# HKUNLP/efficient-attention

Measured on AMD Instinct MI355X. Metric: attn fwd+bwd tokens/s per GPU at N=784, d=64; 1/2/4/8-GPU DDP scaling, higher is better.
Workload: dtype bf16; 1 GPU; lara attention layer fwd+bwd+SGD, x=[128,28,28,192] per GPU (N=784, h=3, d=64), bf16 autocast; attn=lara, global_batch=128, seq_len=784, heads=3, head_dim=64, parallelism=dp1, hipgraph=True, gemm_tunableop=False

## Files before the change

### efficient-attention_amd/csrc/ea_capi.hip

```cpp
#include <stdlib.h>
#include <cmath>
#include "ea_window.h"

namespace ea {
int window_fwd_dispatch(const WinP& p, int dtype, int D, hipStream_t st);
int window_bwd_dispatch(const WinP& p, const ea_geom& geom, const T4& outp, const float* biasT, int dtype, int D,
                        hipStream_t st);
}
#include "ea_landmark_params.h"
#include "ea_lara.h"
#include "ea_softmax.h"
#include "ea_lara_lmk.h"
#include "ea_lara_merge.h"
#include "ea_layernorm.h"
#include "ea_lara_segment.h"
#include "ea_scatter.h"
#include "ea_rows_mlp.h"
#include "ea_performer_f32.h"
#include "ea_kernelized.h"
#include "ea_f32_attn.h"
namespace ea {
int rows_mlp_dispatch(const RowsP& p, int D, int sides, int layer_norm, bool bwd, hipStream_t st);
int rows_mlp_blocks(int R, int D);
int lara_x_dispatch(int mode, const LaraP& p, int dtype, hipStream_t st);
int lara_y_dispatch(int mode, const LaraP& p, int dtype, hipStream_t st);
int lara_f_dispatch(int which, const LaraP& p, int dtype, hipStream_t st);
int pool2d_dispatch(bool bwd, int dtype, const void* x, long sb, long sh, long sn, float* mean, int B, int H, int gh, int gw,
                    int side, int D, hipStream_t st);
int linear_supported(int K, int NO);
int proj_rs_supported(int K, int NO);
int proj_rs_pool_supported(int K, int NO, int B, int gh, int gw, int r);
int proj_rs_dispatch(int dtype, const void* a, int a_f32, const float* w, const float* bias, void* y, void* a_cast, int rows,
                     long lda, long ldy, hipStream_t st, int B, int gh, int gw, int r, float* pq, float* pk, void* w_cast,
                     const void* wsw);
int w192_prepare_dispatch(int dtype, const float* wq, const float* wp, void* w16q, void* wsw, void* w16p, void* w16pT, hipStream_t st);
int dgrad_rs_supported(int K, int NO);
int dgrad_fin_launch(int dtype, const void* dqkv, long ldy, const void* qkv, long ldq, const void* w, int w_f32, void* dx, int dx_f32,
                     long ldx, int B, int gh, int gw, int pool_r, int C, float scale, const float* qbar, const float* uq,
                     const float* lse_t, const float* dpq, const float* dpk, hipStream_t st);
int dgrad_rs_dispatch(int dtype, const void* dy, const void* w, int w_f32, void* dx, int dx_f32, int rows, long ldy, long ldx,
                      hipStream_t st);
int linear_dispatch(int dtype, const void* a, int a_f32, const void* w, int w_mode, const float* bias, void* y, int y_f32,
                    void* a_cast, int rows, int K, int NO, long lda, long ldy, hipStream_t st);
int wgrad_slices(int rows, int M, int K);
int wgrad_pair_slices(int rows, int M1, int K1, int M2, int K2);
int wgrad_pair_dispatch(int dtype, int rows, const void* dy1, const void* x1, float* part1, float* db1, long ld1, int M1, int K1,
                        const void* dy2, const void* x2, float* part2, float* db2, long ld2, int M2, int K2, hipStream_t st);
int wgrad_dispatch(int dtype, const void* dy, const void* x, float* part, float* db_part, long part_ld, int rows, int M,
                   int K, hipStream_t st);
int part_sum_dispatch(const float* part, float* out, int S, int n, long ld, hipStream_t st);
int multi_sum_dispatch(int K, const float* const* part, const int* S, const int* n, const long long* ld, float* const* out,
                       hipStream_t st);
}

using namespace ea;

static bool t4_ok(const ea_t4* t, int D) {
  return t && t->ptr && ((uintptr_t)t->ptr % 16 == 0) && t->sb % 8 == 0 && t->sh % 8 == 0 &&
         t->sn % 8 == 0 && t->sn >= D;
}
static bool t4_ok32(const ea_t4* t, int D, int N) {
  return t4_ok(t, D) && (int64_t)N * t->sn < ((int64_t)1 << 31);
}
static bool geom_ok(const ea_geom* g) {
  return g && g->B > 0 && g->H > 0 && g->N > 0 && (g->D == 32 || g->D == 64 || g->D == 128) &&
         (g->dtype == EA_BF16 || g->dtype == EA_F16) && g->ext >= 0 && g->causal >= 0 && g->causal <= 2 && g->lm_base >= 0;
}
static Geo mk_geo(const ea_geom* g) {
  Geo G;
  G.N = g->N; G.attn2d = g->attn_2d; G.gh = g->attn_2d ? g->gh : 1; G.gw = g->attn_2d ? g->gw : g->N;
  return G;
}

extern "C" {

const char* ea_version(void) { return "ea_hip 0.1.0 gfx950"; }
int32_t ea_abi_version(void) { return 24; }

int32_t ea_window_bias_ld(const ea_geom* g) {
  WinTiling t;
  if (!geom_ok(g) || win_tiling(*g, t, false) != EA_OK) return EA_E_BADARG;
  return t.biasLd;
}
int32_t ea_window_keep_ld(const ea_geom* g) {
  WinTiling t;
  if (!geom_ok(g) || win_tiling(*g, t, false) != EA_OK) return EA_E_BADARG;
  return t.biasLd + t.nCT * 16;
}
int32_t ea_window_bwd_parts(const ea_geom* g) {
  WinTiling t;
  if (!geom_ok(g) || win_tiling(*g, t, true) != EA_OK) return EA_E_BADARG;
  return t.parts_total;
}
int32_t ea_window_bwd_needs_bias_t(const ea_geom* g) {
  WinTiling t;
  if (!geom_ok(g) || win_tiling(*g, t, true) != EA_OK) return EA_E_BADARG;
  int any = 0;
  win_bwd_launches(*g, t, [&](const WinTiling& tl) { any |= window_bwd_lds(tl, g->D, true, true) > WIN_LDS_MAX; });
  return any;
}
int32_t ea_window_bwd_bias_parts(const ea_geom* g) {
  WinTiling t;
  if (!geom_ok(g) || win_tiling(*g, t, true) != EA_OK) return EA_E_BADARG;
  return win_bwd_bias_parts(*g, t);
}
int32_t ea_window_bwd_acc_slices(const ea_geom* g) {
  WinTiling t;
  if (!geom_ok(g) || win_tiling(*g, t, true) != EA_OK) return EA_E_BADARG;
  return win_bwd_acc_slices(t);
}
int32_t ea_window_bwd_query_blocks(const ea_geom* g) {
  WinTiling t;
  if (!geom_ok(g) || win_tiling(*g, t, true) != EA_OK) return EA_E_BADARG;
  return t.qsplit;
}

static int fill_win(const ea_geom* g, WinP& p, bool backward) {
  if (!geom_ok(g)) return EA_E_BADARG;
  int rc = win_tiling(*g, p.t, backward);
  if (rc != EA_OK) return rc;
  if (g->L < 0 || g->L > 64) return EA_E_UNSUPPORTED;
  p.G = mk_geo(g);
  p.B = g->B; p.H = g->H; p.L = g->L; p.w = g->window; p.e = g->ext;
  p.causal = g->causal; p.chunk = g->chunk; p.lm_base = g->causal == 2 ? g->lm_base : 0;
  p.scale = g->scale;
  p.scale_log2 = g->scale * LOG2E;
  return EA_OK;
}

int ea_window_attn_fwd(const ea_geom* g, const ea_t4* q, const ea_t4* k, const ea_t4* v,
                       const float* lk, const float* lv, const float* bias, const uint8_t* mask,
                       const ea_t4* out, float* lse, const uint8_t* keep, float keep_scale, void* stream) {
  WinP p = {};
  int rc = fill_win(g, p, false);
  if (rc != EA_OK) return rc;
  if (keep && !g->causal) return EA_E_UNSUPPORTED;
  p.keep = keep; p.keep_scale = keep_scale; p.keep_ld = p.t.biasLd + p.t.nCT * 16;
  if (!t4_ok(q, g->D) || !t4_ok(k, g->D) || !t4_ok(v, g->D) || !t4_ok(out, g->D) || !lse) return EA_E_BADARG;
  if (g->L > 0 && (!lk || !lv)) return EA_E_BADARG;
  p.q = mk(q); p.k = mk(k); p.v = mk(v); p.o = mk(out);
  p.lk = lk; p.lv = lv; p.bias = bias; p.mask = mask; p.lse = lse;
  return window_fwd_dispatch(p, g->dtype, g->D, (hipStream_t)stream);
}

int ea_window_attn_bwd(const ea_geom* g, const ea_t4* q, const ea_t4* k, const ea_t4* v,
                       const float* lk, const float* lv, const float* bias, const uint8_t* mask,
                       const ea_t4* out, const ea_t4* dout, const float* lse,
                       const ea_t4* dq, const ea_t4* dk, const ea_t4* dv,
                       float* dlk_part, float* dlv_part, float* dbias_part,
                       float* dk_acc, float* dv_acc, const float* bias_t,
                       const uint8_t* keep, float keep_scale, const float* dlse, void* stream) {
  WinP p = {};
  int rc = fill_win(g, p, true);
  if (rc != EA_OK) return rc;
  p.dlse = dlse;
  if (keep && !g->causal) return EA_E_UNSUPPORTED;
  p.keep = keep; p.keep_scale = keep_scale; p.keep_ld = p.t.biasLd + p.t.nCT * 16;
  const int N = g->N;
  if (!t4_ok32(q, g->D, N) || !t4_ok32(k, g->D, N) || !t4_ok32(v, g->D, N) || !t4_ok32(dout, g->D, N) ||
      !t4_ok32(out, g->D, N) || (win_bwd_acc_slices(p.t) > 0 && (!dk_acc || !dv_acc)) || !t4_ok32(dq, g->D, N) ||
// ... 1205 lines not shown
extern "C" {

int32_t ea_linear_supported(int32_t in_features, int32_t out_features) { return linear_supported(in_features, out_features); }

int ea_linear(int32_t dtype, int32_t rows, int32_t in_features, int32_t out_features, const void* a, int32_t a_f32,
              int64_t lda, const void* w, const float* bias, void* y, int32_t y_f32, int64_t ldy, void* a_cast,
              void* stream) {
  if (!a || !w || !y || ((uintptr_t)a & 15) || ((uintptr_t)w & 15) || ((uintptr_t)y & 15) || ((uintptr_t)bias & 15) ||
      ((uintptr_t)a_cast & 15))
    return EA_E_BADARG;
  if (lda < in_features || ldy < out_features || (lda & 7) || (ldy & 7)) return EA_E_BADARG;
  return linear_dispatch(dtype, a, a_f32, w, 0, bias, y, y_f32, a_cast, rows, in_features, out_features, (long)lda,
                         (long)ldy, (hipStream_t)stream);
}

int ea_linear_w32(int32_t dtype, int32_t rows, int32_t in_features, int32_t out_features, const void* a, int32_t a_f32,
                  int64_t lda, const float* w, int32_t w_transposed, const float* bias, void* y, int32_t y_f32, int64_t ldy,
                  void* a_cast, void* stream) {
  if (!a || !w || !y || ((uintptr_t)a & 15) || ((uintptr_t)w & 15) || ((uintptr_t)y & 15) || ((uintptr_t)bias & 15) ||
      ((uintptr_t)a_cast & 15))
    return EA_E_BADARG;
  if (lda < in_features || ldy < out_features || (lda & 7) || (ldy & 7)) return EA_E_BADARG;
  static const bool rs_on = !(getenv("EA_PROJ_RS") && getenv("EA_PROJ_RS")[0] == '0');
  if (rs_on && !w_transposed && !y_f32 && rows >= 65536 && proj_rs_supported(in_features, out_features))
    return proj_rs_dispatch(dtype, a, a_f32, w, bias, y, a_cast, rows, (long)lda, (long)ldy, (hipStream_t)stream, 0, 0, 0, 0,
                            nullptr, nullptr, nullptr, nullptr);
  return linear_dispatch(dtype, a, a_f32, w, w_transposed ? 2 : 1, bias, y, y_f32, a_cast, rows, in_features, out_features,
                         (long)lda, (long)ldy, (hipStream_t)stream);
}

int32_t ea_linear_dgrad_supported(int32_t in_features, int32_t out_features) {
  return dgrad_rs_supported(out_features, in_features);
}

int ea_linear_dgrad(int32_t dtype, int32_t rows, int32_t in_features, int32_t out_features, const void* dy, int64_t ldy,
                    const void* w, int32_t w_f32, void* dx, int32_t dx_f32, int64_t ldx, void* stream) {
  if (!dy || !w || !dx || ((uintptr_t)dy & 15) || ((uintptr_t)w & 15) || ((uintptr_t)dx & 15)) return EA_E_BADARG;
  if (rows < 0 || ldy < out_features || ldx < in_features || (ldy & 7) || (ldx & 3) || (!dx_f32 && (ldx & 7))) return EA_E_BADARG;
  if (!dgrad_rs_supported(out_features, in_features)) return EA_E_UNSUPPORTED;
  if ((int64_t)rows * ldy >= ((int64_t)1 << 40)) return EA_E_BADARG;
  return dgrad_rs_dispatch(dtype, dy, w, w_f32, dx, dx_f32, rows, (long)ldy, (long)ldx, (hipStream_t)stream);
}

int ea_linear_dgrad_finish(int32_t dtype, int32_t B, int32_t gh, int32_t gw, int32_t pool_r, int32_t C, float scale,
                           void* dqkv, int64_t ldy, const void* qkv, int64_t ldq, const void* w, int32_t w_f32, void* dx,
                           int32_t dx_f32, int64_t ldx, const float* qbar, const float* uq, const float* lse_t,
                           const float* dpq, const float* dpk, void* stream) {
  if (!dqkv || !w || !dx || ((uintptr_t)dqkv & 15) || ((uintptr_t)w & 15) || ((uintptr_t)dx & 15) || ((uintptr_t)qkv & 15))
    return EA_E_BADARG;
  if (B <= 0 || gh <= 0 || gw <= 0 || ldy < 576 || ldx < 192 || (ldy & 7) || (ldx & 3) || (!dx_f32 && (ldx & 7))) return EA_E_BADARG;
  if ((dpq == nullptr) != (dpk == nullptr)) return EA_E_BADARG;
  if (dpq && (pool_r <= 0 || gh % pool_r || gw % pool_r)) return EA_E_BADARG;
  if (uq && (!qkv || !qbar || !lse_t || ldq < 192 || (ldq & 7) || C <= 0)) return EA_E_BADARG;
  if (uq && C > 64) return EA_E_UNSUPPORTED;
  if (!uq && !dpq) return EA_E_BADARG;
  if ((int64_t)B * gh * gw >= ((int64_t)1 << 31)) return EA_E_BADARG;
  return dgrad_fin_launch(dtype, dqkv, (long)ldy, qkv, (long)ldq, w, w_f32, dx, dx_f32, (long)ldx, B, gh, gw, pool_r, C, scale,
                          qbar, uq, lse_t, dpq, dpk, (hipStream_t)stream);
}

int32_t ea_linear_pool_supported(int32_t in_features, int32_t out_features, int32_t B, int32_t gh, int32_t gw, int32_t r) {
  return proj_rs_pool_supported(in_features, out_features, B, gh, gw, r);
}

int ea_linear_w32_pool(int32_t dtype, int32_t B, int32_t gh, int32_t gw, int32_t r, int32_t in_features, int32_t out_features,
                       const void* a, int32_t a_f32, int64_t lda, const float* w, const float* bias, void* y, int64_t ldy,
                       void* a_cast, float* pooled_q, float* pooled_k, void* w_cast, void* stream) {
  if (!a || !w || !y || !pooled_q || !pooled_k || ((uintptr_t)a & 15) || ((uintptr_t)w & 15) || ((uintptr_t)y & 15) ||
      ((uintptr_t)bias & 15) || ((uintptr_t)a_cast & 15) || ((uintptr_t)pooled_q & 15) || ((uintptr_t)pooled_k & 15) ||
      ((uintptr_t)w_cast & 15))
    return EA_E_BADARG;
  if (lda < in_features || ldy < out_features || (lda & 7) || (ldy & 7)) return EA_E_BADARG;
  if (!proj_rs_pool_supported(in_features, out_features, B, gh, gw, r)) return EA_E_UNSUPPORTED;
  return proj_rs_dispatch(dtype, a, a_f32, w, bias, y, a_cast, B * gh * gw, (long)lda, (long)ldy, (hipStream_t)stream, B, gh, gw,
                          r, pooled_q, pooled_k, w_cast, nullptr);
}

int ea_linear_w192_prepare(int32_t dtype, const float* wq, const float* wp, void* w16q, void* wq_sw, void* w16p, void* w16pT,
                           void* stream) {
  if (!wq || !w16q || !wq_sw || ((uintptr_t)wq & 15) || ((uintptr_t)wp & 15) || ((uintptr_t)w16q & 15) || ((uintptr_t)wq_sw & 15) ||
      ((uintptr_t)w16p & 15) || ((uintptr_t)w16pT & 15))
    return EA_E_BADARG;
  if (wp && (!w16p || !w16pT)) return EA_E_BADARG;
  return w192_prepare_dispatch(dtype, wq, wp, w16q, wq_sw, w16p, w16pT, (hipStream_t)stream);
}

int ea_linear_wsw(int32_t dtype, int32_t rows, int32_t B, int32_t gh, int32_t gw, int32_t r, const void* a, int32_t a_f32, int64_t lda,
                  const void* wq_sw, const float* bias, void* y, int64_t ldy, void* a_cast, float* pooled_q, float* pooled_k,
                  void* stream) {
  if (!a || !wq_sw || !y || ((uintptr_t)a & 15) || ((uintptr_t)wq_sw & 15) || ((uintptr_t)y & 15) || ((uintptr_t)bias & 15) ||
      ((uintptr_t)a_cast & 15) || ((uintptr_t)pooled_q & 15) || ((uintptr_t)pooled_k & 15))
    return EA_E_BADARG;
  if (lda < 192 || ldy < 576 || (lda & 7) || (ldy & 7) || rows <= 0) return EA_E_BADARG;
  if (r != 0) {
    if (!pooled_q || !pooled_k || rows != B * gh * gw) return EA_E_BADARG;
    if (!proj_rs_pool_supported(192, 576, B, gh, gw, r)) return EA_E_UNSUPPORTED;
  }
  return proj_rs_dispatch(dtype, a, a_f32, nullptr, bias, y, a_cast, rows, (long)lda, (long)ldy, (hipStream_t)stream, B, gh, gw, r,
                          r ? pooled_q : nullptr, r ? pooled_k : nullptr, nullptr, wq_sw);
}

}

static T4s mks(const ea_t4* t) {
  T4s r;
  r.p = t ? (char*)t->ptr : nullptr;
  r.sb = t ? t->sb : 0; r.sh = t ? t->sh : 0; r.sn = t ? t->sn : 0;
  return r;
}
static int fill_sb(const ea_sb_geom* g, SbP& p) {
  if (!g || g->B <= 0 || g->H <= 0 || g->N <= 0 || g->window <= 0 || (g->dtype != EA_BF16 && g->dtype != EA_F16))
    return EA_E_BADARG;
  if (g->D != 64 || g->M <= 0 || g->M > 64) return EA_E_UNSUPPORTED;
  p.B = g->B; p.H = g->H; p.N = g->N; p.M = g->M; p.w = g->window;
  p.G.N = g->N; p.G.attn2d = g->attn_2d; p.G.gh = g->attn_2d ? g->gh : 1; p.G.gw = g->attn_2d ? g->gw : g->N;
  if (g->attn_2d) {
    if (g->gh % g->window || g->gw % g->window || g->gh * g->gw != g->N) return EA_E_BADARG;
    p.Wq = g->window * g->window;
    p.nwin = (g->gh / g->window) * (g->gw / g->window);
  } else {
    if (g->N % g->window) return EA_E_BADARG;
    p.Wq = g->window;
    p.nwin = g->N / g->window;
  }
  if (p.Wq > 64) return EA_E_UNSUPPORTED;
  p.a = 1.f / sqrtf(sqrtf(64.f));
  p.b = 0.5f / sqrtf(64.f);
  p.lconst = 0.5f * logf((float)g->M);
  p.wpb = 1;
  for (int d = 2; d <= 4; ++d)
    if (p.nwin % d == 0) p.wpb = d;
  return EA_OK;
}
static int fill_sb_stats(const ea_sb_geom* g, LaraP& p) {
  ea_perf_geom pg;
  pg.B = g->B; pg.H = g->H; pg.N = g->N; pg.D = g->D; pg.dtype = g->dtype; pg.M = g->M;
  int rc = fill_perf(&pg, p, true);
  if (rc != EA_OK) return rc;
  p.ratio = 1.f; p.feps = 0.f; p.stab_per_feature = 1;
  return EA_OK;
}

extern "C" {

int32_t ea_scatter_parts(const ea_sb_geom* g) {
  LaraP p = {};
  if (!g || fill_sb_stats(g, p) != EA_OK) return EA_E_BADARG;
  return p.nsplit * lara_nsub(p.NCT);
}

int ea_scatter_kmax(const ea_sb_geom* g, const ea_t4* k, const uint8_t* mask, const float* W, float* p_ml, void* stream) {
  LaraP p = {};
  if (!g) return EA_E_BADARG;
  int rc = fill_sb_stats(g, p);
  if (rc != EA_OK) return rc;
  if (!t4_ok(k, g->D) || !W || !p_ml) return EA_E_BADARG;
  p.k = mkl(k); p.mask = mask; p.omega = W; p.p_ml = p_ml;
  return lara_y_dispatch(LY_PMAX, p, g->dtype, (hipStream_t)stream);
}

int ea_scatter_kv(const ea_sb_geom* g, const ea_t4* k, const ea_t4* v, const uint8_t* mask, const float* W,
                  const float* mx, float* p_ml, float* p_kv, void* stream) {
  LaraP p = {};
  if (!g) return EA_E_BADARG;
  int rc = fill_sb_stats(g, p);
  if (rc != EA_OK) return rc;
  if (!t4_ok(k, g->D) || !t4_ok(v, g->D) || !W || !mx || !p_ml || !p_kv) return EA_E_BADARG;
// ... 778 lines not shown
```

### efficient-attention_amd/csrc/ea_common.h

```cpp
#pragma once
#include <hip/hip_runtime.h>
#include <stdint.h>
#include "../../include/ea_hip.h"

#ifdef EA_PROFILE
#include <stdio.h>
#include <algorithm>
#include <vector>
#define EA_STAMP(p, i) do { if (threadIdx.x == 0 && blockIdx.x == 0 && (p).prof) (p).prof[i] = (long long)__builtin_readcyclecounter(); } while (0)
#define EA_BLK(p, e) do { if (threadIdx.x == 0 && (p).prof && blockIdx.x < 8192) (p).prof[128 + 2 * blockIdx.x + (e)] = (long long)wall_clock64(); } while (0)
#define EA_BLKX(p, e) do { if (threadIdx.x == 0 && (p).prof && blockIdx.x < 8192) (p).prof[128 + 2 * 8192 + 2 * blockIdx.x + (e)] = (long long)wall_clock64(); } while (0)
namespace ea {
struct ProfReport {
  static constexpr int NW = 128 + 4 * 8192;
  long long* d = nullptr; hipStream_t st; const char* name; int mode;
  long long* arm(hipStream_t s, const char* nm, int md) {
    static long long* buf = nullptr;
    if (!buf) hipMalloc(&buf, NW * sizeof(long long));
    hipMemsetAsync(buf, 0, NW * sizeof(long long), s);
    d = buf; st = s; name = nm; mode = md;
    return buf;
  }
  ~ProfReport() {
    if (!d) return;
    std::vector<long long> h(NW);
    hipStreamSynchronize(st);
    hipMemcpy(h.data(), d, NW * sizeof(long long), hipMemcpyDeviceToHost);
    fprintf(stderr, "%s mode %d:", name, mode);
    long long prev = h[0];
    for (int i = 1; i < 128; ++i) if (h[i]) { fprintf(stderr, " [%d]%lld", i, h[i] - prev); prev = h[i]; }
    fprintf(stderr, " total %lld\n", prev - h[0]);
    std::vector<long long> b, e, dur;
    for (int i = 0; i < 8192; ++i) if (h[128 + 2 * i] && h[129 + 2 * i]) { b.push_back(h[128 + 2 * i]); e.push_back(h[129 + 2 * i]); dur.push_back(h[129 + 2 * i] - h[128 + 2 * i]); }
    if (!b.empty()) {
      const long long t0 = *std::min_element(b.begin(), b.end());
      std::vector<long long> bs(b), es(e), ds(dur);
      for (auto& x : bs) x -= t0; for (auto& x : es) x -= t0;
      std::sort(bs.begin(), bs.end()); std::sort(es.begin(), es.end()); std::sort(ds.begin(), ds.end());
      const size_t n = bs.size();
      fprintf(stderr, "  %zu blocks (10 ns ticks): start p50 %lld p90 %lld max %lld | dur min %lld p50 %lld p90 %lld max %lld | end p50 %lld max %lld\n",
              n, bs[n / 2], bs[n * 9 / 10], bs[n - 1], ds[0], ds[n / 2], ds[n * 9 / 10], ds[n - 1], es[n / 2], es[n - 1]);
      {
        std::vector<long long> pro, epi;
        for (int i = 0; i < 8192; ++i) {
          const long long b0 = h[128 + 2 * i], e0 = h[129 + 2 * i], x0 = h[128 + 2 * 8192 + 2 * i], x1 = h[129 + 2 * 8192 + 2 * i];
          if (b0 && e0 && x0 && x1) { pro.push_back(x0 - b0); epi.push_back(e0 - x1); }
        }
        if (!pro.empty()) {
          std::sort(pro.begin(), pro.end()); std::sort(epi.begin(), epi.end());
          const size_t m = pro.size();
          fprintf(stderr, "  prologue p10 %lld p50 %lld p90 %lld | epilogue p10 %lld p50 %lld p90 %lld\n", pro[m / 10], pro[m / 2], pro[m * 9 / 10], epi[m / 10], epi[m / 2], epi[m * 9 / 10]);
        }
      }
      fprintf(stderr, "  start deciles:");
      for (int q = 1; q <= 10; ++q) fprintf(stderr, " %lld", bs[(n * q) / 10 - 1]);
      fprintf(stderr, " | dur deciles:");
      for (int q = 1; q <= 10; ++q) fprintf(stderr, " %lld", ds[(n * q) / 10 - 1]);
      fprintf(stderr, " | end deciles:");
      for (int q = 1; q <= 10; ++q) fprintf(stderr, " %lld", es[(n * q) / 10 - 1]);
      fprintf(stderr, "\n");
    }
  }
};
}
#else
#define EA_STAMP(p, i) do { } while (0)
#define EA_BLK(p, e) do { } while (0)
#define EA_BLKX(p, e) do { } while (0)
#endif


namespace ea {

constexpr int EA_MAX_DEV = 64;
inline int ea_cur_device() {
  int dev = 0;
  if (hipGetDevice(&dev) != hipSuccess || dev < 0 || dev >= EA_MAX_DEV) dev = 0;
  return dev;
}
inline int ea_device_cus() {
  static int n[EA_MAX_DEV] = {};
  const int dev = ea_cur_device();
  if (!n[dev]) {
    hipDeviceProp_t prop;
    int v = 0;
    if (hipGetDeviceProperties(&prop, dev) == hipSuccess) v = prop.multiProcessorCount;
// ... 105 lines not shown
template <int G> EA_DEV float group_sum(float v) {
  static_assert(G == 4 || G == 8 || G == 16, "group_sum: 4, 8 or 16 lanes");
  v += dpp_mov<0xB1>(v);
  v += dpp_mov<0x4E>(v);
  if (G >= 8) v += dpp_mov<0x141>(v);
  if (G >= 16) v += dpp_mov<0x128>(v);
  return v;
}
template <int S> EA_DEV float stride_sum(float v) {
  static_assert(S == 4 || S == 8 || S == 16, "stride_sum: stride 4, 8 or 16");
  if (S <= 8) v += dpp_mov<0x128>(v);
  if (S <= 4) v += dpp_mov<0x124>(v);
  return quad_sum(v);
}
template <int S> EA_DEV float stride_max(float v) {
  static_assert(S == 4 || S == 8 || S == 16, "stride_max: stride 4, 8 or 16");
  if (S <= 8) v = fmaxf(v, dpp_mov<0x128>(v));
  if (S <= 4) v = fmaxf(v, dpp_mov<0x124>(v));
  return quad_max(v);
}
EA_DEV float fast_rcp(float x) { return __builtin_amdgcn_rcpf(x); }
EA_DEV float wave_sum(float v) {
#pragma unroll
  for (int o = 32; o > 0; o >>= 1) v += __shfl_xor(v, o);
  return v;
}

static __device__ __attribute__((aligned(64))) char ea_trash[512 * 64];
EA_DEV char* ea_trash_line() { return ea_trash + threadIdx.x * 64; }

#ifdef EA_NT_LOADS
EA_DEV u32x4 ldg16(const void* p) { return __builtin_nontemporal_load(reinterpret_cast<const u32x4*>(p)); }
#else
EA_DEV u32x4 ldg16(const void* p) { return *reinterpret_cast<const u32x4*>(p); }
#endif
#ifdef EA_NT_STORES
EA_DEV void stg16(void* p, u32x4 v) { __builtin_nontemporal_store(v, reinterpret_cast<u32x4*>(p)); }
#else
EA_DEV void stg16(void* p, u32x4 v) { *reinterpret_cast<u32x4*>(p) = v; }
#endif
EA_DEV u32x4 lds16(const char* p) { return *reinterpret_cast<const u32x4*>(p); }
EA_DEV void sts16(char* p, u32x4 v) { *reinterpret_cast<u32x4*>(p) = v; }

struct Geo {
  int N, attn2d, gh, gw;
};
EA_DEV int part_token(const Geo& G, int part, int slot, int side, int ext) {
  if (G.attn2d) {
    const int t = side + 2 * ext;
    const int per_row = G.gw / side;
    const int p1 = part / per_row, p2 = part - p1 * per_row;
    const int i = slot / t, j = slot - i * t;
    const int y = p1 * side - ext + i, x = p2 * side - ext + j;
    return (y >= 0 && y < G.gh && x >= 0 && x < G.gw) ? y * G.gw + x : -1;
  }
  const int tok = part * side - ext + slot;
  return (tok >= 0 && tok < G.N) ? tok : -1;
}

template <int D> EA_DEV int lds_off(int row, int chunk16) {
  constexpr int CPR = D / 8;
  constexpr int SW = CPR >= 8 ? 7 : CPR - 1;
  return row * (D * 2) + ((chunk16 ^ (row & SW)) << 4);
}

template <int D> struct LaneOff {
  static constexpr int ROWB = D * 2, CPR = D / 8, KS = D / 32, DT = D / 16, DQ = D / 4;
  static constexpr int SW = CPR >= 8 ? 7 : CPR - 1;
  int plain[KS];
  int tr[DT];
  EA_DEV void init(int lane) {
    const int g = lane >> 4, li = lane & 15;
#pragma unroll
    for (int ks = 0; ks < KS; ++ks) plain[ks] = li * ROWB + (((g * KS + ks) ^ (li & SW)) << 4);
    const int r = 4 * g + (li >> 2);
#pragma unroll
    for (int dt = 0; dt < DT; ++dt) {
      const int colb = (DQ * (li & 3) + 4 * dt) * 2;
      tr[dt] = r * ROWB + ((((colb >> 4)) ^ (r & SW)) << 4) + (colb & 15);
    }
  }
};

EA_DEV int phi2(int row) { return (((row >> 1) & 3) << 1) | ((row ^ (row >> 3)) & 1); }
template <int D> EA_DEV int lds_off2(int row, int chunk16) {
  static_assert(D == 64, "lds_off2: 128-byte rows only");
  return row * (D * 2) + ((chunk16 ^ phi2(row)) << 4);
}
template <int D> struct LaneOff2 {
  static constexpr int ROWB = D * 2, KS = D / 32, DT = D / 16;
  int plain[KS];
  int tr[DT];
  EA_DEV void init(int lane) {
    const int g = lane >> 4, li = lane & 15;
#pragma unroll
    for (int ks = 0; ks < KS; ++ks) plain[ks] = lds_off2<D>(li, g * KS + ks);
    const int r = 4 * g + (li >> 2);
#pragma unroll
    for (int dt = 0; dt < DT; ++dt) tr[dt] = lds_off2<D>(r, 2 * dt + ((li & 3) >> 1)) + 8 * (li & 1);
  }
};
template <int W> EA_DEV void quad_transpose(uint32_t (&x)[4][W]);
template <> EA_DEV void quad_transpose<2>(uint32_t (&x)[4][2]) {
  asm volatile("s_nop 15\n\tv_permlane32_swap_b32 %0, %4\n\tv_permlane32_swap_b32 %2, %6\n\t"
               "v_permlane32_swap_b32 %1, %5\n\tv_permlane32_swap_b32 %3, %7"
               : "+v"(x[0][0]), "+v"(x[0][1]), "+v"(x[1][0]), "+v"(x[1][1]), "+v"(x[2][0]), "+v"(x[2][1]), "+v"(x[3][0]), "+v"(x[3][1]));
  asm volatile("s_nop 1\n\tv_permlane16_swap_b32 %0, %2\n\tv_permlane16_swap_b32 %4, %6\n\t"
               "v_permlane16_swap_b32 %1, %3\n\tv_permlane16_swap_b32 %5, %7"
               : "+v"(x[0][0]), "+v"(x[0][1]), "+v"(x[1][0]), "+v"(x[1][1]), "+v"(x[2][0]), "+v"(x[2][1]), "+v"(x[3][0]), "+v"(x[3][1]));
}
template <> EA_DEV void quad_transpose<4>(uint32_t (&x)[4][4]) {
  asm volatile("s_nop 15\n\t"
               "v_permlane32_swap_b32 %0, %8\n\tv_permlane32_swap_b32 %4, %12\n\t"
               "v_permlane32_swap_b32 %1, %9\n\tv_permlane32_swap_b32 %5, %13\n\t"
               "v_permlane32_swap_b32 %2, %10\n\tv_permlane32_swap_b32 %6, %14\n\t"
               "v_permlane32_swap_b32 %3, %11\n\tv_permlane32_swap_b32 %7, %15"
               : "+v"(x[0][0]), "+v"(x[0][1]), "+v"(x[0][2]), "+v"(x[0][3]), "+v"(x[1][0]), "+v"(x[1][1]), "+v"(x[1][2]), "+v"(x[1][3]),
                 "+v"(x[2][0]), "+v"(x[2][1]), "+v"(x[2][2]), "+v"(x[2][3]), "+v"(x[3][0]), "+v"(x[3][1]), "+v"(x[3][2]), "+v"(x[3][3]));
  asm volatile("s_nop 1\n\t"
               "v_permlane16_swap_b32 %0, %4\n\tv_permlane16_swap_b32 %8, %12\n\t"
               "v_permlane16_swap_b32 %1, %5\n\tv_permlane16_swap_b32 %9, %13\n\t"
               "v_permlane16_swap_b32 %2, %6\n\tv_permlane16_swap_b32 %10, %14\n\t"
               "v_permlane16_swap_b32 %3, %7\n\tv_permlane16_swap_b32 %11, %15"
               : "+v"(x[0][0]), "+v"(x[0][1]), "+v"(x[0][2]), "+v"(x[0][3]), "+v"(x[1][0]), "+v"(x[1][1]), "+v"(x[1][2]), "+v"(x[1][3]),
                 "+v"(x[2][0]), "+v"(x[2][1]), "+v"(x[2][2]), "+v"(x[2][3]), "+v"(x[3][0]), "+v"(x[3][1]), "+v"(x[3][2]), "+v"(x[3][3]));
}
EA_DEV void quad_transpose_f32(const f32x4* acc, float* f) {
  uint32_t x[4][4];
#pragma unroll
  for (int s = 0; s < 4; ++s)
#pragma unroll
    for (int r = 0; r < 4; ++r) {
      const float t = acc[s][r];
      x[s][r] = __builtin_bit_cast(uint32_t, t);
    }
  quad_transpose<4>(x);
#pragma unroll
  for (int s = 0; s < 4; ++s)
#pragma unroll
    for (int r = 0; r < 4; ++r) f[4 * s + r] = __builtin_bit_cast(float, x[s][r]);
}
template <typename E> EA_DEV void quad_transpose_pack(const f32x4* acc, float mul, u32x4& o0, u32x4& o1) {
  uint32_t x[4][2];
#pragma unroll
  for (int s = 0; s < 4; ++s) {
    x[s][0] = pack2<E>(acc[s][0] * mul, acc[s][1] * mul);
    x[s][1] = pack2<E>(acc[s][2] * mul, acc[s][3] * mul);
  }
  quad_transpose<2>(x);
  o0 = u32x4{x[0][0], x[0][1], x[1][0], x[1][1]};
  o1 = u32x4{x[2][0], x[2][1], x[3][0], x[3][1]};
}

template <int D> struct TileL {
  static constexpr bool NEWTR = (D == 64);
  static EA_DEV int off(int row, int chunk16) {
    if constexpr (NEWTR) return lds_off2<D>(row, chunk16);
    else return lds_off<D>(row, chunk16);
  }
};
template <int D> EA_DEV int tile_tr(int r, int li, int dt) {
  const int colb = TileL<D>::NEWTR ? (16 * dt + 4 * (li & 3)) * 2 : ((D / 4) * (li & 3) + 4 * dt) * 2;
  return TileL<D>::off(r, colb >> 4) + (colb & 15);
}
template <int D> struct LaneOffSel { typedef LaneOff<D> type; };
template <> struct LaneOffSel<64> { typedef LaneOff2<64> type; };
template <int D> EA_DEV int acc_chan(int dt, int g) { return TileL<D>::NEWTR ? 16 * dt + 4 * g : (D / 4) * g + 4 * dt; }

}
```

### efficient-attention_amd/csrc/ea_dgrad_rs.hip

```cpp
#include <stdlib.h>
#include "ea_common.h"

namespace ea {

struct DgP {
  const char* dy;
  const char* w;
  char* dx;
  int rows, ntiles;
  long ldy, ldx;
  long long* prof;
};

constexpr int DG_K = 576, DG_NO = 192, DG_WAVES = 12, DG_TOK = 32, DG_KT = DG_K / 32, DG_SLABS = DG_K / 64;
constexpr int DG_TILE = DG_SLABS * DG_TOK * 128;
constexpr int DG_PIECE = 32 * DG_NO * 2;
constexpr int DG_LDS = 2 * DG_TILE;

EA_DEV int dg_off(int slab, int tok, int chunk16) { return slab * (DG_TOK * 128) + lds_off2<64>(tok, chunk16); }

template <typename E, bool WF32, bool OF32>
__global__ __launch_bounds__(DG_WAVES * 64, 3) void dgrad_rs_kernel(const DgP p) {
  extern __shared__ __attribute__((aligned(16))) char smem[];
  char* const tile0 = smem;
  char* const tile1 = smem + DG_TILE;
  const int tid = threadIdx.x, lane = tid & 63, g = lane >> 4, li = lane & 15;
  const int wave = __builtin_amdgcn_readfirstlane(tid >> 6);
  int s_tok[3], s_ch[3];
#pragma unroll
  for (int i = 0; i < 3; ++i) {
    const int s = tid + i * (DG_WAVES * 64);
    s_tok[i] = s / 72;
    s_ch[i] = s - s_tok[i] * 72;
  }
  u32x4 nb[3];
  auto issue = [&](int t) {
#pragma unroll
    for (int i = 0; i < 3; ++i) {
      const int tok = min(t * DG_TOK + s_tok[i], p.rows - 1);
      nb[i] = ldg16(p.dy + ((size_t)tok * p.ldy + s_ch[i] * 8) * 2);
    }
  };
  int t = blockIdx.x;
  if (t < p.ntiles) issue(t);
  typename E::x8 wr[DG_KT];
  {
    const int o_l = tid / 24, c = tid - o_l * 24;
    const int rho = ((o_l >> 2) & 1) * 16 + (o_l >> 3) * 4 + (o_l & 3);
    const int wofs = rho * (DG_NO * 2) + c * 16;
    const int rofs = (4 * g + (li >> 2)) * (DG_NO * 2) + (16 * wave + 4 * (li & 3)) * 2;
    constexpr int BATCH = 6;
#pragma unroll
    for (int pb = 0; pb < DG_KT; pb += BATCH) {
      u32x4 raw[BATCH][WF32 ? 2 : 1];
#pragma unroll
      for (int j = 0; j < BATCH; ++j) {
        const size_t e = (size_t)(32 * (pb + j) + o_l) * DG_NO + c * 8;
        if constexpr (WF32) {
          raw[j][0] = ldg16(p.w + e * 4);
          raw[j][1] = ldg16(p.w + e * 4 + 16);
        } else {
          raw[j][0] = ldg16(p.w + e * 2);
        }
      }
#pragma unroll
      for (int j = 0; j < BATCH; ++j) {
        u32x4 w8;
        if constexpr (WF32) {
          const f32x4 lo = __builtin_bit_cast(f32x4, raw[j][0]), hi = __builtin_bit_cast(f32x4, raw[j][1]);
          const float f[8] = {lo[0], lo[1], lo[2], lo[3], hi[0], hi[1], hi[2], hi[3]};
          w8 = pack8<E>(f);
        } else {
          w8 = raw[j][0];
        }
        char* img = tile1 + ((pb + j) & 1) * DG_PIECE;
        sts16(img + wofs, w8);
        __syncthreads();
        wr[pb + j] = as_x8<E>(E::tr4(img + rofs), E::tr4(img + rofs + 16 * (DG_NO * 2)));
      }
    }
  }
  int buf = 0;
  for (; t < p.ntiles; t += gridDim.x, buf ^= 1) {
    char* const tb = buf ? tile1 : tile0;
#pragma unroll
    for (int i = 0; i < 3; ++i) sts16(tb + dg_off(s_ch[i] >> 3, s_tok[i], s_ch[i] & 7), nb[i]);
    issue(min(t + (int)gridDim.x, p.ntiles - 1));
    __syncthreads();
    f32x4 acc[2][2];
#pragma unroll
    for (int rt = 0; rt < 2; ++rt) acc[rt][0] = acc[rt][1] = f32x4{0.f, 0.f, 0.f, 0.f};
#pragma unroll
    for (int ks = 0; ks < DG_KT; ++ks) {
      const int slab = ks >> 1;
      const typename E::x8 b0 = as_x8<E>(lds16(tb + dg_off(slab, li, 4 * (ks & 1) + g)));
      const typename E::x8 b1 = as_x8<E>(lds16(tb + dg_off(slab, 16 + li, 4 * (ks & 1) + g)));
      acc[0][ks & 1] = E::mma(wr[ks], b0, acc[0][ks & 1]);
      acc[1][ks & 1] = E::mma(wr[ks], b1, acc[1][ks & 1]);
    }
#pragma unroll
    for (int rt = 0; rt < 2; ++rt) {
      const int tok = min(t * DG_TOK + 16 * rt + li, p.rows - 1);
      const f32x4 v = acc[rt][0] + acc[rt][1];
      const int col = 16 * wave + 4 * g;
      if constexpr (OF32) {
        *reinterpret_cast<f32x4*>(p.dx + ((size_t)tok * p.ldx + col) * 4) = v;
      } else {
        *reinterpret_cast<u32x2*>(p.dx + ((size_t)tok * p.ldx + col) * 2) = u32x2{pack2<E>(v[0], v[1]), pack2<E>(v[2], v[3])};
      }
    }
  }
}

struct DgFinP {
  DgP d;
  const char* qkv;
  long ldq;
  const float *qbar, *uq, *lse_t;
  const float *dpq, *dpk;
  int ntok, gw, pool_r, cw, L, C;
  float pool_inv, scale, scale_log2;
  int splits, tps, nunits;
  unsigned m_gw, m_r;
  int cps;
  unsigned m_cw;
};

constexpr int DG_QT = 3 * DG_TOK * 128;
constexpr int DG_LMR = 64 * 128;
constexpr int DG_FIN_LDS = 2 * DG_TILE + 2 * DG_QT + 6 * DG_LMR + 3 * 64 * 4;

template <typename E, bool WF32, bool OF32, bool HAS_T, bool POOL, int PR>
__global__ __launch_bounds__(DG_WAVES * 64, 3) void dgrad_fin_kernel(const DgFinP p) {
  static_assert(PR == 0 || (POOL && (PR == 2 || PR == 4)), "cell-major order needs 2 x 2 or 4 x 4 pooling cells");
  constexpr int TPC = PR * PR, CPT = PR ? DG_TOK / (PR * PR) : 1;
  extern __shared__ __attribute__((aligned(16))) char smem[];
  char* const tile0 = smem;
  char* const tile1 = smem + DG_TILE;
  char* const qt0 = smem + 2 * DG_TILE;
  char* const R1 = qt0 + 2 * DG_QT;
  char* const R2 = R1 + 3 * DG_LMR;
  float* const LS = reinterpret_cast<float*>(R2 + 3 * DG_LMR);
  const int tid = threadIdx.x, lane = tid & 63, g = lane >> 4, li = lane & 15;
  const int wave = __builtin_amdgcn_readfirstlane(tid >> 6);
  constexpr bool pool = POOL;
  EA_BLK(p.d, 0);
  typename E::x8 wr[DG_KT];
  {
    const int o_l = tid / 24, c = tid - o_l * 24;
    const int rho = ((o_l >> 2) & 1) * 16 + (o_l >> 3) * 4 + (o_l & 3);
    const int wofs = rho * (DG_NO * 2) + c * 16;
    const int rofs = (4 * g + (li >> 2)) * (DG_NO * 2) + (16 * wave + 4 * (li & 3)) * 2;
    constexpr int BATCH = 6;
#pragma unroll
    for (int pb = 0; pb < DG_KT; pb += BATCH) {
      u32x4 raw[BATCH][WF32 ? 2 : 1];
#pragma unroll
      for (int j = 0; j < BATCH; ++j) {
        const size_t e = (size_t)(32 * (pb + j) + o_l) * DG_NO + c * 8;
        if constexpr (WF32) {
          raw[j][0] = ldg16(p.d.w + e * 4);
          raw[j][1] = ldg16(p.d.w + e * 4 + 16);
        } else {
          raw[j][0] = ldg16(p.d.w + e * 2);
        }
      }
#pragma unroll
      for (int j = 0; j < BATCH; ++j) {
        u32x4 w8;
        if constexpr (WF32) {
          const f32x4 lo = __builtin_bit_cast(f32x4, raw[j][0]), hi = __builtin_bit_cast(f32x4, raw[j][1]);
          const float f[8] = {lo[0], lo[1], lo[2], lo[3], hi[0], hi[1], hi[2], hi[3]};
          w8 = pack8<E>(f);
        } else {
          w8 = raw[j][0];
        }
        char* img = tile1 + ((pb + j) & 1) * DG_PIECE;
        sts16(img + wofs, w8);
        __syncthreads();
        wr[pb + j] = as_x8<E>(E::tr4(img + rofs), E::tr4(img + rofs + 16 * (DG_NO * 2)));
      }
    }
  }
  typename LaneOffSel<64>::type lo;
  lo.init(lane);
  const int fh = wave >> 2, fnt = (wave >> 1) & 1, fdh = wave & 1;
  int buf = 0;
  EA_BLKX(p.d, 0);
  for (int u = blockIdx.x; u < p.nunits; u += gridDim.x) {
    const int b = u / p.splits, sp = u - b * p.splits;
    const int n0 = PR ? sp * p.cps : sp * p.tps, n1 = PR ? min(p.L, n0 + p.cps) : min(p.ntok, n0 + p.tps);
    const size_t row0 = (size_t)b * p.ntok;
    const int ntile = PR ? (n1 - n0 + CPT - 1) / CPT : (n1 - n0 + DG_TOK - 1) / DG_TOK;
    auto slot_cell = [&](int t, int r) { return min(n0 + t * CPT + r / (TPC ? TPC : 1), n1 - 1); };
    auto dup = [&](int t, int r) {
      if constexpr (PR == 0) return n0 + t * DG_TOK + r > n1 - 1;
      else return n0 + t * CPT + r / (TPC ? TPC : 1) > n1 - 1;
    };
    auto trash_line = [&]() {
      int t_ = tid;
      asm volatile("" : "+v"(t_));
      return ea_trash + (t_ & 511) * 64;
    };
    auto tok_of = [&](int t, int r) {
      if constexpr (PR == 0) {
        return min(n0 + t * DG_TOK + r, n1 - 1);
      } else {
        const int cell = slot_cell(t, r), w = r % TPC;
        const int cy = (int)__umulhi((unsigned)cell, p.m_cw), cx = cell - cy * p.cw;
        return (cy * PR + w / PR) * p.gw + cx * PR + w % PR;
      }
    };
    auto cell_of_tok = [&](int tok) {
      const int y = (int)__umulhi((unsigned)tok, p.m_gw), x = tok - y * p.gw;
      return (int)__umulhi((unsigned)y, p.m_r) * p.cw + (int)__umulhi((unsigned)x, p.m_r);
    };
    auto cell_of = [&](int t, int r) {
      if constexpr (PR == 0) return cell_of_tok(tok_of(t, r));
      else return slot_cell(t, r);
    };
    u32x4 nb[3], nq;
    f32x4 npk[2], npq[2];
    auto issue = [&](int t, int s_tok, int s_c) {
      const int tok = tok_of(t, s_tok);
      const char* rowp = p.d.dy + ((row0 + tok) * p.d.ldy + s_c * 8) * 2;
      nb[0] = ldg16(rowp);
      nb[1] = ldg16(rowp + 192 * 2);
      nb[2] = ldg16(rowp + 384 * 2);
      if constexpr (HAS_T) nq = ldg16(p.qkv + ((row0 + tok) * p.ldq + s_c * 8) * 2);
#ifdef EA_DGF_NOPOOLREAD
      npk[0] = npk[1] = npq[0] = npq[1] = f32x4{0.f, 0.f, 0.f, 0.f};
// ... 82 lines not shown
        const float* src = p.dpq + ((size_t)(b * 3 + fh) * p.L + cell_of(t, 16 * fnt + li)) * 64 + 4 * g;
#pragma unroll
        for (int j = 0; j < 2; ++j) pq4[j] = *reinterpret_cast<const f32x4*>(src + 16 * (2 * fdh + j));
      }
      issue(min(t + 1, ntile - 1), s_tok, s_c);
      __syncthreads();
      if constexpr (HAS_T) {
        const char* R1h = R1 + fh * DG_LMR;
        const char* R2h = R2 + fh * DG_LMR;
        const float* LSh = LS + fh * 64;
        typename E::x8 f1[2];
#pragma unroll
        for (int ks = 0; ks < 2; ++ks) f1[ks] = as_x8<E>(lds16(qb + dg_off(fh, 16 * fnt + li, g * 2 + ks)));
        f32x4 acc[2] = {f32x4{0.f, 0.f, 0.f, 0.f}, f32x4{0.f, 0.f, 0.f, 0.f}};
#pragma unroll
        for (int kk = 0; kk < 2; ++kk) {
          uint32_t pw[4];
#pragma unroll
          for (int c2 = 0; c2 < 2; ++c2) {
            const int ct = 2 * kk + c2;
            f32x4 tt = {0.f, 0.f, 0.f, 0.f};
#pragma unroll
            for (int ks = 0; ks < 2; ++ks) tt = E::mma(as_x8<E>(lds16(R2h + TileL<64>::off(ct * 16 + li, g * 2 + ks))), f1[ks], tt);
            const f32x4 ls = *reinterpret_cast<const f32x4*>(LSh + ct * 16 + 4 * g);
            pw[2 * c2] = pack2<E>(fast_exp2(tt[0] * p.scale_log2 - ls[0]), fast_exp2(tt[1] * p.scale_log2 - ls[1]));
            pw[2 * c2 + 1] = pack2<E>(fast_exp2(tt[2] * p.scale_log2 - ls[2]), fast_exp2(tt[3] * p.scale_log2 - ls[3]));
          }
          const u32x4 p1 = {pw[0], pw[1], pw[2], pw[3]};
#pragma unroll
          for (int j = 0; j < 2; ++j) {
            const char* r1 = R1h + (32 * kk) * 128 + (fdh ? lo.tr[2 + j] : lo.tr[j]);
            acc[j] = E::mma(as_x8<E>(E::tr4(r1), E::tr4(r1 + 16 * 128)), as_x8<E>(p1), acc[j]);
          }
        }
#pragma unroll
        for (int j = 0; j < 2; ++j) {
          const int dt = 2 * fdh + j;
          char* a = tb + dg_off(fh, 16 * fnt + li, 2 * dt + (g >> 1)) + (g & 1) * 8;
          const u32x2 old = *reinterpret_cast<const u32x2*>(a);
          float o4[4];
          unpack2<E>(old[0], o4[0], o4[1]);
          unpack2<E>(old[1], o4[2], o4[3]);
#pragma unroll
          for (int r = 0; r < 4; ++r) o4[r] = o4[r] - acc[j][r] * p.scale + pq4[j][r] * p.pool_inv;
          *reinterpret_cast<u32x2*>(a) = u32x2{pack2<E>(o4[0], o4[1]), pack2<E>(o4[2], o4[3])};
        }
        __syncthreads();
        stg16(dup(t, s_tok) ? trash_line() : const_cast<char*>(p.d.dy) + ((row0 + tok_of(t, s_tok)) * p.d.ldy + s_c * 8) * 2,
              lds16(tb + dg_off(s_c >> 3, s_tok, s_c & 7)));
      }
      f32x4 acc[2][2];
#pragma unroll
      for (int rt = 0; rt < 2; ++rt) acc[rt][0] = acc[rt][1] = f32x4{0.f, 0.f, 0.f, 0.f};
#pragma unroll
      for (int ks = 0; ks < DG_KT; ++ks) {
        const int slab = ks >> 1;
        const typename E::x8 b0 = as_x8<E>(lds16(tb + dg_off(slab, li, 4 * (ks & 1) + g)));
        const typename E::x8 b1 = as_x8<E>(lds16(tb + dg_off(slab, 16 + li, 4 * (ks & 1) + g)));
        acc[0][ks & 1] = E::mma(wr[ks], b0, acc[0][ks & 1]);
        acc[1][ks & 1] = E::mma(wr[ks], b1, acc[1][ks & 1]);
      }
      int li_x = lane;
      asm volatile("" : "+v"(li_x));
      li_x &= 15;
#pragma unroll
      for (int rt = 0; rt < 2; ++rt) {
        const size_t row = row0 + tok_of(t, 16 * rt + li_x);
        const bool dpx = dup(t, 16 * rt + li_x);
        const f32x4 v = acc[rt][0] + acc[rt][1];
        const int col = 16 * wave + 4 * g;
        if constexpr (OF32) {
          *reinterpret_cast<f32x4*>(dpx ? trash_line() : p.d.dx + (row * p.d.ldx + col) * 4) = v;
        } else {
          *reinterpret_cast<u32x2*>(dpx ? trash_line() : p.d.dx + (row * p.d.ldx + col) * 2) = u32x2{pack2<E>(v[0], v[1]), pack2<E>(v[2], v[3])};
        }
      }
    }
    if constexpr (HAS_T) __syncthreads();
  }
  EA_BLKX(p.d, 1);
  EA_BLK(p.d, 1);
}

int dgrad_rs_supported(int K, int NO) { return K == DG_K && NO == DG_NO; }

int dgrad_rs_dispatch(int dtype, const void* dy, const void* w, int w_f32, void* dx, int dx_f32, int rows, long ldy, long ldx,
                      hipStream_t st) {
  if (rows <= 0) return EA_OK;
  DgP p = {};
  p.dy = (const char*)dy; p.w = (const char*)w; p.dx = (char*)dx;
  p.rows = rows; p.ntiles = (rows + DG_TOK - 1) / DG_TOK; p.ldy = ldy; p.ldx = ldx;
  int grid = ea_device_cus();
  if (grid > p.ntiles) grid = p.ntiles;
  const dim3 g((unsigned)grid), b(DG_WAVES * 64);
#define EA_DG_LAUNCH(E_, WF_, OF_)                                                        \
  do {                                                                                    \
    EA_SET_LDS_ONCE((&dgrad_rs_kernel<E_, WF_, OF_>), DG_LDS);                            \
    hipLaunchKernelGGL((dgrad_rs_kernel<E_, WF_, OF_>), g, b, DG_LDS, st, p);             \
  } while (0)
#define EA_DG_SEL(E_)                                                                     \
  do {                                                                                    \
    if (w_f32) { if (dx_f32) EA_DG_LAUNCH(E_, true, true); else EA_DG_LAUNCH(E_, true, false); }   \
    else { if (dx_f32) EA_DG_LAUNCH(E_, false, true); else EA_DG_LAUNCH(E_, false, false); }       \
  } while (0)
  if (dtype == EA_BF16) EA_DG_SEL(BF16);
  else if (dtype == EA_F16) EA_DG_SEL(F16);
  else return EA_E_BADARG;
#undef EA_DG_SEL
#undef EA_DG_LAUNCH
  return (int)hipGetLastError();
}

int dgrad_fin_dispatch(int dtype, const DgFinP& p0, int w_f32, int dx_f32, bool has_t, int pr, hipStream_t st) {
  DgFinP p = p0;
  if (p.d.rows <= 0) return EA_OK;
  int grid = ea_device_cus();
  if (grid > p.nunits) grid = p.nunits;
  const dim3 g((unsigned)grid), b(DG_WAVES * 64);
#ifdef EA_PROFILE
  ProfReport rep;
  p.d.prof = rep.arm(st, "dgrad_fin", pr);
#endif
#define EA_DF_LAUNCH(E_, WF_, OF_, T_, P_, R_)                                                    \
  do {                                                                                            \
    EA_SET_LDS_ONCE((&dgrad_fin_kernel<E_, WF_, OF_, T_, P_, R_>), DG_FIN_LDS);                   \
    hipLaunchKernelGGL((dgrad_fin_kernel<E_, WF_, OF_, T_, P_, R_>), g, b, DG_FIN_LDS, st, p);    \
  } while (0)
#define EA_DF_SEL3(E_, WF_, OF_, T_)                                                          \
  do {                                                                                        \
    if (pr == 4) EA_DF_LAUNCH(E_, WF_, OF_, T_, true, 4);                                     \
    else if (pr == 2) EA_DF_LAUNCH(E_, WF_, OF_, T_, true, 2);                                \
    else EA_DF_LAUNCH(E_, WF_, OF_, T_, true, 0);                                             \
  } while (0)
#define EA_DF_SEL2(E_, WF_, OF_)                                                              \
  do {                                                                                        \
    if (has_t && p.dpq) EA_DF_SEL3(E_, WF_, OF_, true);                                       \
    else if (has_t) EA_DF_LAUNCH(E_, WF_, OF_, true, false, 0);                               \
    else EA_DF_SEL3(E_, WF_, OF_, false);                                                     \
  } while (0)
#define EA_DF_SEL(E_)                                                                     \
  do {                                                                                    \
    if (w_f32) { if (dx_f32) EA_DF_SEL2(E_, true, true); else EA_DF_SEL2(E_, true, false); }   \
    else { if (dx_f32) EA_DF_SEL2(E_, false, true); else EA_DF_SEL2(E_, false, false); }       \
  } while (0)
  if (dtype == EA_BF16) EA_DF_SEL(BF16);
  else if (dtype == EA_F16) EA_DF_SEL(F16);
  else return EA_E_BADARG;
#undef EA_DF_SEL
#undef EA_DF_SEL2
#undef EA_DF_SEL3
#undef EA_DF_LAUNCH
  return (int)hipGetLastError();
}

int dgrad_fin_launch(int dtype, const void* dqkv, long ldy, const void* qkv, long ldq, const void* w, int w_f32, void* dx, int dx_f32,
                     long ldx, int B, int gh, int gw, int pool_r, int C, float scale, const float* qbar, const float* uq,
                     const float* lse_t, const float* dpq, const float* dpk, hipStream_t st) {
  DgFinP p = {};
  p.d.dy = (const char*)dqkv; p.d.w = (const char*)w; p.d.dx = (char*)dx;
  p.ntok = gh * gw;
  p.d.rows = B * p.ntok; p.d.ntiles = 0; p.d.ldy = ldy; p.d.ldx = ldx;
  p.qkv = (const char*)qkv; p.ldq = ldq;
  p.qbar = qbar; p.uq = uq; p.lse_t = lse_t; p.dpq = dpq; p.dpk = dpk;
  p.gw = gw; p.pool_r = dpq ? pool_r : 1; p.cw = gw / p.pool_r; p.L = (gh / p.pool_r) * p.cw; p.C = C;
  p.pool_inv = 1.f / (float)(p.pool_r * p.pool_r); p.scale = scale; p.scale_log2 = scale * LOG2E;
  p.m_gw = (unsigned)((1ull << 32) / (unsigned)gw) + 1u; p.m_r = (unsigned)((1ull << 32) / (unsigned)p.pool_r) + 1u;
  const int cus = ea_device_cus();
  int splits = (cus + B - 1) / B;
  if (splits < 1) splits = 1;
  int tps = ((p.ntok + splits - 1) / splits + DG_TOK - 1) / DG_TOK * DG_TOK;
  if (tps < 2 * DG_TOK) tps = 2 * DG_TOK;
  p.tps = tps;
  p.splits = (p.ntok + tps - 1) / tps;
  static const bool cells_on = !(getenv("EA_DGF_CELLS") && getenv("EA_DGF_CELLS")[0] == '0');
  int pr = 0;
  if (dpq && cells_on && (pool_r == 2 || pool_r == 4) && gh % pool_r == 0 && gw % pool_r == 0) {
    pr = pool_r;
    const int cpt = DG_TOK / (pr * pr);
    int cps = ((p.L + splits - 1) / splits + cpt - 1) / cpt * cpt;
    if (cps < 2 * cpt) cps = 2 * cpt;
    p.cps = cps;
    p.splits = (p.L + cps - 1) / cps;
    p.m_cw = (unsigned)((1ull << 32) / (unsigned)p.cw) + 1u;
  }
  p.nunits = B * p.splits;
  return dgrad_fin_dispatch(dtype, p, w_f32, dx_f32, uq != nullptr, pr, st);
}

}
```

### efficient-attention_amd/csrc/ea_proj_rs.hip

```cpp
#include "ea_common.h"

namespace ea {

struct RsP {
  const char* a;
  const float* w;
  const float* bias;
  char* y;
  char* a_cast;
  char* w_cast;
  int rows, ntiles;
  long lda, ldy;
  float *pq, *pk;
  int gw, cw, Lc, ntok, ncell;
  unsigned m_Lc, m_cw;
  long long* prof;
  const char* wsw;
};

constexpr int RS_K = 192, RS_NO = 576, RS_WAVES = 12, RS_TOK = 32, RS_KT = RS_K / 32, RS_SLABS = RS_K / 64;

EA_DEV int rs_off(int slab, int tok, int chunk16) { return slab * (RS_TOK * 128) + lds_off2<64>(tok, chunk16); }

EA_DEV int rs_col(int wave, int j, int li) {
  const int c0 = 48 * wave;
  return j == 2 ? c0 + 32 + li : c0 + 8 * (li >> 2) + (li & 3) + 4 * j;
}

template <typename E, bool AF32, int POOL, bool WSW>
__global__ __launch_bounds__(RS_WAVES * 64, 3) void proj_rs_kernel(const RsP p) {
  __shared__ __attribute__((aligned(16))) char tile[2][RS_SLABS * RS_TOK * 128];
  __shared__ __attribute__((aligned(16))) float bias_s[RS_NO];
  const int tid = threadIdx.x, lane = tid & 63, g = lane >> 4, li = lane & 15;
  const int wave = __builtin_amdgcn_readfirstlane(tid >> 6);
  const int st_tok = tid / 24, st_c = tid - st_tok * 24;
  constexpr int PR = POOL == 16 ? 4 : 2;
  auto cell_of = [&](int t, int s, int& img, int& cl) {
    const int cell = min(t * (RS_TOK / (POOL ? POOL : 1)) + s / (POOL ? POOL : 1), p.ncell - 1);
    img = (int)__umulhi((unsigned)cell, p.m_Lc);
    cl = cell - img * p.Lc;
  };
  auto tok_of = [&](int t, int s) {
    if constexpr (POOL == 0) {
      return min(t * RS_TOK + s, p.rows - 1);
    } else {
      int img, cl;
      cell_of(t, s, img, cl);
      const int cy = (int)__umulhi((unsigned)cl, p.m_cw), cx = cl - cy * p.cw;
      const int w = s % POOL, dy = w / PR, dx = w % PR;
      return img * p.ntok + (cy * PR + dy) * p.gw + cx * PR + dx;
    }
  };
  u32x4 nb[AF32 ? 2 : 1];
  auto issue = [&](int t) {
    const int tok = tok_of(t, st_tok);
    const char* ap = p.a + (size_t)tok * p.lda * (AF32 ? 4 : 2) + st_c * (AF32 ? 32 : 16);
    nb[0] = ldg16(ap);
    if constexpr (AF32) nb[1] = ldg16(ap + 16);
  };
  int t = blockIdx.x;
  EA_BLK(p, 0);
  if (t < p.ntiles) issue(t);
  typename E::x8 wr[3][RS_KT];
  for (int i = tid; i < RS_NO; i += RS_WAVES * 64) bias_s[i] = p.bias ? E::to_f(E::from_f(p.bias[i])) : 0.f;
  if constexpr (WSW) {
#pragma unroll
    for (int j = 0; j < 3; ++j)
#pragma unroll
      for (int ks = 0; ks < RS_KT; ++ks)
        wr[j][ks] = as_x8<E>(ldg16(p.wsw + ((size_t)((wave * 3 + j) * RS_KT + ks) * 64 + lane) * 16));
  } else {
    const int col[3] = {rs_col(wave, 0, li), rs_col(wave, 1, li), rs_col(wave, 2, li)};
#pragma unroll
    for (int j = 0; j < 3; ++j)
#pragma unroll
      for (int ks = 0; ks < RS_KT; ++ks) {
        const float* s = p.w + (size_t)col[j] * RS_K + ks * 32 + 8 * g;
        const f32x4 lo = *reinterpret_cast<const f32x4*>(s), hi = *reinterpret_cast<const f32x4*>(s + 4);
        const float f[8] = {lo[0], lo[1], lo[2], lo[3], hi[0], hi[1], hi[2], hi[3]};
        wr[j][ks] = as_x8<E>(pack8<E>(f));
        if (p.w_cast && (unsigned)((wave * 3 + j) * RS_KT + ks) % gridDim.x == blockIdx.x)
          stg16(p.w_cast + ((size_t)col[j] * RS_K + ks * 32 + 8 * g) * 2, __builtin_bit_cast(u32x4, wr[j][ks]));
      }
  }
  const int slab_s = st_c >> 3, ch_s = st_c & 7;
  constexpr int NC = POOL ? RS_TOK / POOL : 1;
  constexpr int XB = 8 * RS_K * 2;
  __shared__ __attribute__((aligned(16))) char xbar[POOL ? 2 : 1][POOL ? 2 * XB : 16];
  const int pc0 = 48 * wave;
  auto pool_x = [&](int b_) {
    const int slab = wave >> 2, dt = wave & 3;
    const char* tb = tile[b_] + slab * (RS_TOK * 128);
    const int r_ = 4 * g + (li >> 2);
    const int off = lds_off2<64>(r_, 2 * dt + ((li & 3) >> 1)) + 8 * (li & 1);
    const typename E::x8 a = as_x8<E>(E::tr4(tb + off), E::tr4(tb + 16 * 128 + off));
    const uint32_t one = (uint32_t)E::from_f(1.f) * 0x00010001u;
    const uint32_t lo_on = (POOL == 16 ? li == 0 : li == g) ? one : 0u, hi_on = (POOL == 16 ? li == 1 : li == 4 + g) ? one : 0u;
    const typename E::x8 pat = as_x8<E>(u32x4{lo_on, lo_on, hi_on, hi_on});
    const f32x4 d = E::mma(a, pat, f32x4{0.f, 0.f, 0.f, 0.f});
    float hi[4], lo[4];
#pragma unroll
    for (int r = 0; r < 4; ++r) {
      const float v = d[r] * (1.f / (POOL ? POOL : 1));
      hi[r] = E::to_f(E::from_f(v));
      lo[r] = v - hi[r];
    }
    if (li < NC) {
      char* dst = xbar[b_] + li * (RS_K * 2) + (64 * slab + 16 * dt + 4 * g) * 2;
      *reinterpret_cast<u32x2*>(dst) = u32x2{pack2<E>(hi[0], hi[1]), pack2<E>(hi[2], hi[3])};
      *reinterpret_cast<u32x2*>(dst + XB) = u32x2{pack2<E>(lo[0], lo[1]), pack2<E>(lo[2], lo[3])};
    }
  };
  auto pool_out = [&](int tp, int b_) {
    if (wave >= 8) return;
    f32x4 pa[3] = {f32x4{0.f, 0.f, 0.f, 0.f}, f32x4{0.f, 0.f, 0.f, 0.f}, f32x4{0.f, 0.f, 0.f, 0.f}};
    const char* xb = xbar[b_] + min(li, NC - 1) * (RS_K * 2);
#pragma unroll
    for (int ks = 0; ks < RS_KT; ++ks) {
      const typename E::x8 bh = as_x8<E>(lds16(xb + (4 * ks + g) * 16));
      const typename E::x8 bl = as_x8<E>(lds16(xb + XB + (4 * ks + g) * 16));
#pragma unroll
      for (int j = 0; j < 3; ++j) {
        pa[j] = E::mma(wr[j][ks], bh, pa[j]);
        pa[j] = E::mma(wr[j][ks], bl, pa[j]);
      }
    }
    const int cell = tp * NC + li;
    if (li < NC && cell < p.ncell) {
      const int img = (int)__umulhi((unsigned)cell, p.m_Lc), cl = cell - img * p.Lc;
      const int cols[3] = {pc0 + 8 * g, pc0 + 8 * g + 4, pc0 + 32 + 4 * g};
#pragma unroll
      for (int j = 0; j < 3; ++j) {
        const int side = wave >> 2, hc = cols[j] - side * RS_K, head = hc >> 6, ch = hc & 63;
        float* dst = (side ? p.pk : p.pq) + ((size_t)(img * 3 + head) * p.Lc + cl) * 64 + ch;
        *reinterpret_cast<f32x4*>(dst) = pa[j] + *reinterpret_cast<const f32x4*>(bias_s + cols[j]);
      }
    }
  };
  int buf = 0, tprev = -1;
  EA_BLKX(p, 0);
  for (; t < p.ntiles; tprev = t, t += gridDim.x, buf ^= 1) {
    {
      u32x4 w8;
      if constexpr (AF32) {
        const f32x4 lo = __builtin_bit_cast(f32x4, nb[0]), hi = __builtin_bit_cast(f32x4, nb[1]);
        const float f[8] = {lo[0], lo[1], lo[2], lo[3], hi[0], hi[1], hi[2], hi[3]};
        w8 = pack8<E>(f);
      } else {
        w8 = nb[0];
      }
      sts16(tile[buf] + rs_off(slab_s, st_tok, ch_s), w8);
      if (AF32 && p.a_cast) {
        const int tok = tok_of(t, st_tok);
        stg16(p.a_cast + ((size_t)tok * RS_K + st_c * 8) * 2, w8);
      }
    }
    if (t + (int)gridDim.x < p.ntiles) issue(t + gridDim.x);
    __syncthreads();
#ifndef EA_RS_NOPOOLMATH
    if constexpr (POOL > 0) pool_x(buf);
#endif
    f32x4 acc[3][2];
#pragma unroll
    for (int j = 0; j < 3; ++j) acc[j][0] = acc[j][1] = f32x4{0.f, 0.f, 0.f, 0.f};
#pragma unroll
    for (int ks = 0; ks < RS_KT; ++ks) {
      const int slab = ks >> 1;
      const typename E::x8 b0 = as_x8<E>(lds16(tile[buf] + rs_off(slab, li, 4 * (ks & 1) + g)));
      const typename E::x8 b1 = as_x8<E>(lds16(tile[buf] + rs_off(slab, 16 + li, 4 * (ks & 1) + g)));
#pragma unroll
      for (int j = 0; j < 3; ++j) {
        acc[j][0] = E::mma(wr[j][ks], b0, acc[j][0]);
        acc[j][1] = E::mma(wr[j][ks], b1, acc[j][1]);
      }
    }
    const int c0 = 48 * wave;
    const f32x4 bv0 = *reinterpret_cast<const f32x4*>(bias_s + c0 + 8 * g), bv1 = *reinterpret_cast<const f32x4*>(bias_s + c0 + 8 * g + 4);
    const f32x4 bv2 = *reinterpret_cast<const f32x4*>(bias_s + c0 + 32 + 4 * g);
    u32x2 third[2];
#pragma unroll
    for (int rt = 0; rt < 2; ++rt) {
      const int tok = tok_of(t, 16 * rt + li);
      char* yp = p.y + ((size_t)tok * p.ldy + c0) * 2;
      const f32x4 v0 = acc[0][rt] + bv0, v1 = acc[1][rt] + bv1, v2 = acc[2][rt] + bv2;
      u32x4 o;
      o[0] = pack2<E>(v0[0], v0[1]); o[1] = pack2<E>(v0[2], v0[3]);
      o[2] = pack2<E>(v1[0], v1[1]); o[3] = pack2<E>(v1[2], v1[3]);
      stg16(yp + 16 * g, o);
      third[rt] = u32x2{pack2<E>(v2[0], v2[1]), pack2<E>(v2[2], v2[3])};
    }
    asm volatile("s_nop 1\n\tv_permlane16_swap_b32 %0, %2\n\tv_permlane16_swap_b32 %1, %3"
                 : "+v"(third[0][0]), "+v"(third[0][1]), "+v"(third[1][0]), "+v"(third[1][1]));
    {
      const int tok = tok_of(t, 16 * (g & 1) + li);
      const u32x4 o = {third[0][0], third[0][1], third[1][0], third[1][1]};
      stg16(p.y + ((size_t)tok * p.ldy + c0 + 32 + 8 * (g >> 1)) * 2, o);
    }
#ifndef EA_RS_NOPOOLMATH
    if constexpr (POOL > 0) {
      if (tprev >= 0) pool_out(tprev, buf ^ 1);
    }
#endif
  }
  EA_BLKX(p, 1);
  if constexpr (POOL > 0) {
    if (tprev >= 0) {
      __syncthreads();
      pool_out(tprev, buf ^ 1);
    }
  }
  EA_BLK(p, 1);
}

int proj_rs_supported(int K, int NO) { return K == RS_K && NO == RS_NO; }

static unsigned rs_magic(int d) { return (unsigned)((1ull << 32) / (unsigned)d) + 1u; }

int proj_rs_pool_supported(int K, int NO, int B, int gh, int gw, int r) {
  if (K != RS_K || NO != RS_NO || (r != 2 && r != 4) || B <= 0 || gh <= 0 || gw <= 0 || gh % r || gw % r) return 0;
  const long Lc = (long)(gh / r) * (gw / r), ncell = (long)B * Lc;
  return ncell * Lc < (1l << 32) && (long)B * gh * gw < (1l << 31);
}

template <typename E>
__global__ __launch_bounds__(256) void w192_prepare_kernel(const float* __restrict__ wq, const float* __restrict__ wp,
                                                            char* __restrict__ w16q, char* __restrict__ wsw,
                                                            char* __restrict__ w16p, char* __restrict__ w16pT) {
  constexpr int NQ = RS_WAVES * 3 * RS_KT * 64, NP = RS_K * RS_K / 8;
  const int i = blockIdx.x * 256 + threadIdx.x;
  if (i < NQ) {
    const int lane = i & 63, pc = i >> 6, ks = pc % RS_KT, wj = pc / RS_KT, j = wj % 3, wave = wj / 3;
    const int g = lane >> 4, li = lane & 15;
    const size_t e = (size_t)rs_col(wave, j, li) * RS_K + ks * 32 + 8 * g;
    const f32x4 lo = *reinterpret_cast<const f32x4*>(wq + e), hi = *reinterpret_cast<const f32x4*>(wq + e + 4);
    const float f[8] = {lo[0], lo[1], lo[2], lo[3], hi[0], hi[1], hi[2], hi[3]};
    const u32x4 w8 = pack8<E>(f);
    stg16(wsw + (size_t)i * 16, w8);
    stg16(w16q + e * 2, w8);
  } else if (i < NQ + NP && wp) {
    const int k = i - NQ, row = k / (RS_K / 8), c = k - row * (RS_K / 8);
    const size_t e = (size_t)row * RS_K + c * 8;
    const f32x4 lo = *reinterpret_cast<const f32x4*>(wp + e), hi = *reinterpret_cast<const f32x4*>(wp + e + 4);
    const float f[8] = {lo[0], lo[1], lo[2], lo[3], hi[0], hi[1], hi[2], hi[3]};
    const u32x4 w8 = pack8<E>(f);
    stg16(w16p + e * 2, w8);
    uint16_t* t = reinterpret_cast<uint16_t*>(w16pT);
#pragma unroll
    for (int q = 0; q < 4; ++q) {
      t[(size_t)(c * 8 + 2 * q) * RS_K + row] = (uint16_t)(w8[q] & 0xffffu);
      t[(size_t)(c * 8 + 2 * q + 1) * RS_K + row] = (uint16_t)(w8[q] >> 16);
    }
  }
}

int w192_prepare_dispatch(int dtype, const float* wq, const float* wp, void* w16q, void* wsw, void* w16p, void* w16pT,
                          hipStream_t st) {
  constexpr int N = RS_WAVES * 3 * RS_KT * 64 + RS_K * RS_K / 8;
  const dim3 g((N + 255) / 256), b(256);
  if (dtype == EA_BF16) hipLaunchKernelGGL(w192_prepare_kernel<BF16>, g, b, 0, st, wq, wp, (char*)w16q, (char*)wsw, (char*)w16p, (char*)w16pT);
  else if (dtype == EA_F16) hipLaunchKernelGGL(w192_prepare_kernel<F16>, g, b, 0, st, wq, wp, (char*)w16q, (char*)wsw, (char*)w16p, (char*)w16pT);
  else return EA_E_BADARG;
  return (int)hipGetLastError();
}

int proj_rs_dispatch(int dtype, const void* a, int a_f32, const float* w, const float* bias, void* y, void* a_cast, int rows,
                     long lda, long ldy, hipStream_t st, int B, int gh, int gw, int r, float* pq, float* pk, void* w_cast,
                     const void* wsw) {
  if (rows <= 0) return EA_OK;
  RsP p = {};
  p.a = (const char*)a; p.w = w; p.bias = bias; p.y = (char*)y; p.a_cast = a_f32 ? (char*)a_cast : nullptr;
  p.w_cast = wsw ? nullptr : (char*)w_cast;
  p.wsw = (const char*)wsw;
  p.rows = rows; p.ntiles = (rows + RS_TOK - 1) / RS_TOK; p.lda = lda; p.ldy = ldy;
  const int pool = r * r;
  if (pool) {
    if (!pq || !pk || rows != B * gh * gw) return EA_E_BADARG;
    p.pq = pq; p.pk = pk; p.gw = gw; p.cw = gw / r; p.Lc = (gh / r) * p.cw; p.ntok = gh * gw; p.ncell = B * p.Lc;
    p.m_Lc = rs_magic(p.Lc); p.m_cw = rs_magic(p.cw);
    p.ntiles = (p.ncell * pool + RS_TOK - 1) / RS_TOK;
  }
  int grid = ea_device_cus();
  if (grid > p.ntiles) grid = p.ntiles;
  const dim3 g((unsigned)grid), b(RS_WAVES * 64);
#ifdef EA_PROFILE
  ProfReport rep;
  p.prof = rep.arm(st, "proj_rs", pool);
#endif
#define EA_RS_LAUNCH2(E_, AF_, W_)                                                                             \
  do {                                                                                                         \
    if (pool == 16) hipLaunchKernelGGL((proj_rs_kernel<E_, AF_, 16, W_>), g, b, 0, st, p);                     \
    else if (pool == 4) hipLaunchKernelGGL((proj_rs_kernel<E_, AF_, 4, W_>), g, b, 0, st, p);                  \
    else hipLaunchKernelGGL((proj_rs_kernel<E_, AF_, 0, W_>), g, b, 0, st, p);                                 \
  } while (0)
#define EA_RS_LAUNCH(E_, AF_)                                                                                  \
  do {                                                                                                         \
    if (p.wsw) EA_RS_LAUNCH2(E_, AF_, true);                                                                   \
    else EA_RS_LAUNCH2(E_, AF_, false);                                                                        \
  } while (0)
  if (dtype == EA_BF16) {
    if (a_f32) EA_RS_LAUNCH(BF16, true);
    else EA_RS_LAUNCH(BF16, false);
  } else if (dtype == EA_F16) {
    if (a_f32) EA_RS_LAUNCH(F16, true);
    else EA_RS_LAUNCH(F16, false);
  } else {
    return EA_E_BADARG;
  }
#undef EA_RS_LAUNCH
#undef EA_RS_LAUNCH2
  return (int)hipGetLastError();
}

}
```

### efficient-attention_amd/efficient_attention/_native.py

```python
import ctypes
import os

import torch

_HERE = os.path.dirname(os.path.abspath(__file__))
_LIB_PATH = os.environ.get(
    "EA_HIP_LIB", os.path.join(os.path.dirname(_HERE), "lib", "libea_hip.so"))

EA_BF16, EA_F16, EA_F32 = 0, 1, 2
_DTYPES = {torch.bfloat16: EA_BF16, torch.float16: EA_F16}


class ea_t4(ctypes.Structure):
    _fields_ = [("ptr", ctypes.c_void_p), ("sb", ctypes.c_int64), ("sh", ctypes.c_int64),
                ("sn", ctypes.c_int64)]


ABI_VERSION = 24


class ea_geom(ctypes.Structure):
    _fields_ = [("B", ctypes.c_int32), ("H", ctypes.c_int32), ("N", ctypes.c_int32),
                ("D", ctypes.c_int32), ("dtype", ctypes.c_int32), ("attn_2d", ctypes.c_int32),
                ("gh", ctypes.c_int32), ("gw", ctypes.c_int32), ("window", ctypes.c_int32),
                ("ext", ctypes.c_int32), ("chunk", ctypes.c_int32), ("L", ctypes.c_int32),
                ("scale", ctypes.c_float), ("causal", ctypes.c_int32), ("lm_base", ctypes.c_int32)]


class ea_perf_geom(ctypes.Structure):
    _fields_ = [("B", ctypes.c_int32), ("H", ctypes.c_int32), ("N", ctypes.c_int32),
                ("D", ctypes.c_int32), ("dtype", ctypes.c_int32), ("M", ctypes.c_int32)]


class ea_kz_geom(ctypes.Structure):
    _fields_ = [("B", ctypes.c_int32), ("H", ctypes.c_int32), ("N", ctypes.c_int32), ("D", ctypes.c_int32),
                ("dtype", ctypes.c_int32), ("map", ctypes.c_int32), ("M", ctypes.c_int32), ("F", ctypes.c_int32),
                ("nu", ctypes.c_int32), ("cos", ctypes.c_int32)]


class ea_sb_geom(ctypes.Structure):
    _fields_ = [("B", ctypes.c_int32), ("H", ctypes.c_int32), ("N", ctypes.c_int32), ("D", ctypes.c_int32),
                ("dtype", ctypes.c_int32), ("M", ctypes.c_int32), ("attn_2d", ctypes.c_int32),
                ("gh", ctypes.c_int32), ("gw", ctypes.c_int32), ("window", ctypes.c_int32)]


class ea_lmk_geom(ctypes.Structure):
    _fields_ = [("BH", ctypes.c_int32), ("L", ctypes.c_int32), ("C", ctypes.c_int32), ("D", ctypes.c_int32),
                ("has_mlp", ctypes.c_int32), ("mixed", ctypes.c_int32), ("mis", ctypes.c_int32),
                ("dup", ctypes.c_int32), ("scale", ctypes.c_float), ("eva", ctypes.c_int32)]


class ea_lara_layer(ctypes.Structure):
    _fields_ = [("B", ctypes.c_int32), ("H", ctypes.c_int32), ("D", ctypes.c_int32), ("dtype", ctypes.c_int32),
                ("gh", ctypes.c_int32), ("gw", ctypes.c_int32), ("pool_r", ctypes.c_int32),
                ("has_mlp", ctypes.c_int32), ("mixed", ctypes.c_int32), ("mis", ctypes.c_int32), ("dup", ctypes.c_int32),
                ("kappa", ctypes.c_float), ("scale", ctypes.c_float)]


class ea_f32_attn(ctypes.Structure):
    _fields_ = [("B", ctypes.c_int32), ("H", ctypes.c_int32), ("Nq", ctypes.c_int32), ("Nk", ctypes.c_int32), ("D", ctypes.c_int32),
                ("G", ctypes.c_int32), ("Wq", ctypes.c_int32), ("Wk", ctypes.c_int32), ("L", ctypes.c_int32),
                ("knorm", ctypes.c_int32), ("neg_inf", ctypes.c_int32), ("causal_e", ctypes.c_int32), ("chunk", ctypes.c_int32),
                ("lm_base", ctypes.c_int32), ("bias_ld", ctypes.c_int32), ("bias_hs", ctypes.c_int64), ("bias_bs", ctypes.c_int64),
                ("keep_ld", ctypes.c_int64),
                ("keep_scale", ctypes.c_float), ("scale", ctypes.c_float)]


class ea_ceva_dec_geom(ctypes.Structure):
    _fields_ = [("B", ctypes.c_int32), ("H", ctypes.c_int32), ("D", ctypes.c_int32), ("dtype", ctypes.c_int32),
                ("window", ctypes.c_int32), ("ext", ctypes.c_int32), ("chunk", ctypes.c_int32), ("t0", ctypes.c_int32),
                ("T_new", ctypes.c_int32), ("c_first", ctypes.c_int32), ("c_last", ctypes.c_int32), ("cap", ctypes.c_int32),
                ("adaptive", ctypes.c_int32), ("has_bias", ctypes.c_int32), ("has_mask", ctypes.c_int32)]


class ea_ceva_sdec_geom(ctypes.Structure):
    _fields_ = [("B", ctypes.c_int32), ("H", ctypes.c_int32), ("D", ctypes.c_int32), ("dtype", ctypes.c_int32),
                ("window", ctypes.c_int32), ("ext", ctypes.c_int32), ("chunk", ctypes.c_int32), ("T_new", ctypes.c_int32),
                ("cap", ctypes.c_int32), ("adaptive", ctypes.c_int32), ("has_bias", ctypes.c_int32), ("ring", ctypes.c_int32),
                ("pos", ctypes.c_void_p), ("status", ctypes.c_void_p), ("ntok", ctypes.c_void_p)]


class ea_eva_layer(ctypes.Structure):
    _fields_ = [("B", ctypes.c_int32), ("H", ctypes.c_int32), ("D", ctypes.c_int32), ("dtype", ctypes.c_int32),
                ("gh", ctypes.c_int32), ("gw", ctypes.c_int32), ("window", ctypes.c_int32), ("chunk", ctypes.c_int32),
                ("has_bias", ctypes.c_int32), ("scale", ctypes.c_float)]


class ea_lara_geom(ctypes.Structure):
    _fields_ = [("B", ctypes.c_int32), ("H", ctypes.c_int32), ("N", ctypes.c_int32),
                ("D", ctypes.c_int32), ("dtype", ctypes.c_int32), ("C", ctypes.c_int32),
                ("mis", ctypes.c_int32), ("kappa", ctypes.c_float), ("scale", ctypes.c_float)]


_P = ctypes.c_void_p
_I = ctypes.c_int32
_L = ctypes.c_int64
_F = ctypes.c_float
_G = ctypes.POINTER(ea_geom)
_LG = ctypes.POINTER(ea_lara_geom)
_PG = ctypes.POINTER(ea_perf_geom)
_KG = ctypes.POINTER(ea_kz_geom)
_MG = ctypes.POINTER(ea_lmk_geom)
_T = ctypes.POINTER(ea_t4)
_SG = ctypes.POINTER(ea_sb_geom)
_LL = ctypes.POINTER(ea_lara_layer)
_EL = ctypes.POINTER(ea_eva_layer)
_FA = ctypes.POINTER(ea_f32_attn)
_DG = ctypes.POINTER(ea_ceva_dec_geom)
_SDG = ctypes.POINTER(ea_ceva_sdec_geom)

SIGNATURES = {
    "ea_eva_chunk_mean_fwd": [_G, _T, _T, _P, _P, _P, _P],
    "ea_eva_chunk_mean_bwd": [_G, _P, _P, _P, _T, _T, _P],
    "ea_eva_beta_fwd": [_G, _T, _T, _P, _P, _P, _P],
    "ea_eva_beta_bwd": [_G, _T, _T, _P, _P, _P, _P, _T, _T, _P, _P],
    "ea_window_attn_fwd": [_G, _T, _T, _T, _P, _P, _P, _P, _T, _P, _P, _F, _P],
    "ea_window_attn_bwd": [_G, _T, _T, _T, _P, _P, _P, _P, _T, _T, _P, _T, _T, _T, _P, _P, _P, _P, _P, _P, _P, _F, _P, _P],
    "ea_window_keep_ld": [_G],
    "ea_rows_mlp_parts": [_I, _I],
    "ea_rows_mlp_fwd": [_I] * 4 + [_P] * 15,
    "ea_rows_mlp_bwd": [_I] * 4 + [_P] * 15,
    "ea_lara_landmarks_fwd": [_MG] + [_P] * 17,
    "ea_lara_landmarks_bwd": [_MG] + [_P] * 21,
    "ea_lara_landmarks_bwd_parts": [_MG] + [_P] * 12 + [_I, _P, _F] + [_P] * 9,
    "ea_lara_out_fwd_merge": [_LG, _T, _P, _P, _P, _I, _P, _P, _P, _P, _P, _P, _P, _T, _P, _P, _P],
    "ea_lara_bwd_k_fused_merge": [_LG, _T, _T, _P, _P, _P, _P, _P, _I, _P, _P, _P, _P, _P, _T, _T, _P, _P, _P, _P, _P, _P, _P],
    "ea_lara_landmarks_fwd_cb": [_MG] + [_P] * 18,
    "ea_lara_landmarks_bwd_cb": [_MG] + [_P] * 23,
    "ea_lara_landmarks_saved_floats": [_MG],
    "ea_lara_merge_fwd": [_I] * 5 + [_P] * 8,
    "ea_lara_merge_bwd": [_I] * 5 + [_F] + [_P] * 16,
    "ea_bias_grad_parts": [_I, _I],
    "ea_bias_grad": [_I, _I, _I, _P, _P, _P, _P],
    "ea_colsum_f32": [_I, _I, _P, _P, _P],
    "ea_colsum2_f32": [_I, _I, _P, _P, _I, _P, _P, _P],
    "ea_slice_sum": [_I, _I, _I, _F, _P, _P, _P, _P],
    "ea_stream_copy": [_P, _P, _L, _P],
    "ea_lara_segment_fwd": [_G, _T, _T] + [_P] * 12,
    "ea_lara_segment_bwd": [_G, _T, _T] + [_P] * 11 + [_T, _T, _P, _P],
    "ea_lara_parts": [_LG],
    "ea_lara_stats_fwd": [_LG, _T, _T, _T, _P, _P, _P, _P, _P, _P],
    "ea_lara_out_fwd": [_LG, _T, _P, _P, _P, _P, _P, _P, _T, _P, _P, _P],
    "ea_lara_bwd_q": [_LG, _T, _T, _P, _P, _P, _P, _P, _P, _T, _P, _P, _P, _P, _P],
    "ea_lara_bwd_qstats": [_LG, _T, _T] + [_P] * 16,
    "ea_lara_bwd_k": [_LG, _T, _T, _P, _P, _P, _P, _P, _P, _T, _T, _P],
    "ea_lara_bwd_kstats": [_LG, _T, _T] + [_P] * 8,
    "ea_lara_bwd_qcorr": [_LG, _T, _P, _P, _P, _T, _P],
    "ea_lara_fused_parts": [_LG],
    "ea_lara_bwd_q_fused": [_LG, _T, _T, _P, _P, _P, _P, _P, _P, _P, _P, _T, _P, _P, _P, _P, _P, _P],
    "ea_lara_bwd_k_fused": [_LG, _T, _T, _P, _P, _P, _P, _P, _P, _T, _T, _P, _P],
    "ea_lara_bwd_finish": [_LG, _T, _P, _P, _P, _P, _P, _I, _I, _I, _T, _T, _P],
    "ea_lara_sample_fwd": [_I, _I, _I, _I, _I, _I, _F] + [_P] * 8,
    "ea_lara_sample_bwd": [_I, _I, _I, _I, _I, _I, _F] + [_P] * 10,
    "ea_adaptive_pool2d_fwd": [_I, _I, _I, _I, _I, _I, _I, _T, _P, _P],
    "ea_adaptive_pool2d_bwd": [_I, _I, _I, _I, _I, _I, _I, _P, _T, _P],
    "ea_gather_sum": [_I, _I, _I, _P, _P, _P, _P],
    "ea_table_bias_fwd": [_I, _I, _I, _I, _I, _F, _P, _P, _P, _P],
    "ea_multi_cast": [_I, _I, _P, _P, _P, _P],
    "ea_linear_w192_prepare": [_I, _P, _P, _P, _P, _P, _P, _P],
    "ea_linear_wsw": [_I, _I, _I, _I, _I, _I, _P, _I, _L, _P, _P, _P, _L, _P, _P, _P, _P],
    "ea_table_bias_bwd": [_I, _I, _I, _I, _I, _I, _F, _P, _P, _P, _P],
    "ea_linear_supported": [_I, _I],
    "ea_linear": [_I, _I, _I, _I, _P, _I, _L, _P, _P, _P, _I, _L, _P, _P],
    "ea_linear_w32": [_I, _I, _I, _I, _P, _I, _L, _P, _I, _P, _P, _I, _L, _P, _P],
    "ea_linear_pool_supported": [_I] * 6,
    "ea_f32_attn_fwd": [_FA, _T, _T, _T, _T, _T, _P, _P, _P, _P, _P, _P, _T, _P, _P, _P],
    "ea_f32_attn_bwd": [_FA, _T, _T, _T, _T, _T, _P, _P, _P, _P, _P, _P, _T, _T, _P, _P, _T, _P, _P, _P, _P, _P, _P],
    "ea_f32_gather_mean_fwd": [_I, _I, _I, _I, _I, _I, _T, _P, _P, _P, _P],
    "ea_f32_gather_mean_bwd": [_I, _I, _I, _I, _I, _I, _P, _P, _P, _P, _P],
    "ea_linear_dgrad_supported": [_I, _I],
    "ea_linear_dgrad": [_I, _I, _I, _I, _P, _L, _P, _I, _P, _I, _L, _P],
    "ea_linear_dgrad_finish": [_I, _I, _I, _I, _I, _I, _F, _P, _L, _P, _L, _P, _I, _P, _I, _L, _P, _P, _P, _P, _P, _P],
    "ea_linear_w32_pool": [_I] * 7 + [_P, _I, _L, _P, _P, _P, _L, _P, _P, _P, _P, _P],
    "ea_wgrad_parts": [_I, _I, _I],
    "ea_wgrad": [_I, _I, _I, _I, _P, _P, _P, _P, _L, _P],
    "ea_wgrad_pair_parts": [_I, _I, _I, _I, _I],
    "ea_layernorm_parts": [_I],
    "ea_layernorm_fwd": [_I, _I, _I, _P, _P, _P, _F, _P, _P, _P],
    "ea_layernorm_bwd": [_I, _I, _I, _P, _P, _P, _P, _P, _P, _P],
    "ea_wgrad_pair": [_I, _I, _I, _I, _P, _P, _P, _P, _L, _I, _I, _P, _P, _P, _P, _L, _P],
    "ea_part_sum": [_I, _I, _L, _P, _P, _P],
    "ea_multi_sum": [_I, _P, _P, _P, _P, _P, _P],
    "ea_lara_layer_ws": [_LL, _I],
    "ea_lara_layer_fwd": [_LL, _T, _T, _T, _P, _P, _P, _T, _P, _P, _I, _P],
    "ea_lara_layer_bwd": [_LL, _T, _T, _T, _P, _P, _P, _T, _T, _T, _T, _P, _P, _P, _P],
    "ea_lara_layer_bwd2": [_LL, _T, _T, _T, _P, _P, _P, _T, _T, _T, _T, _P, _P, _P, _I, _P],
    "ea_eva_layer_ws": [_EL, _I],
    "ea_eva_layer_fwd": [_EL, _T, _T, _T, _P, _P, _P, _T, _P, _I, _P],
    "ea_eva_layer_bwd": [_EL, _T, _T, _T, _P, _P, _P, _T, _T, _T, _T, _T, _P, _P, _P, _P, _P],
    "ea_eva_layer_bwd2": [_EL, _T, _T, _T, _P, _P, _P, _T, _T, _T, _T, _T, _P, _P, _P, _P, _I, _P],
    "ea_scatter_parts": [_SG],
    "ea_scatter_kmax": [_SG, _T, _P, _P, _P, _P],
    "ea_scatter_kv": [_SG, _T, _T, _P, _P, _P, _P, _P, _P],
    "ea_scatter_fwd": [_SG, _T, _T, _T, _P, _P, _P, _P, _P, _T, _P, _T, _P, _P],
    "ea_scatter_bwd_parts": [_SG],
    "ea_scatter_bwd_window": [_SG, _T, _T, _T, _P, _P, _P, _P, _P, _T, _P, _P, _T, _T, _T, _T, _T, _P, _P, _P, _P],
    "ea_scatter_bwd_global": [_SG, _T, _T, _P, _P, _P, _P, _P, _T, _T, _P],
    "ea_scatter_ov_windows": [_SG, _I],
    "ea_scatter_ov_fwd": [_SG, _I, _T, _T, _T, _P, _P, _P, _P, _P, _T, _P, _T, _P, _P],
    "ea_scatter_ov_bwd_window": [_SG, _I, _T, _T, _T, _P, _P, _P, _P, _P, _T, _P, _P, _T, _T, _T, _P, _P, _P, _P, _P],
    "ea_scatter_ov_bwd_keys": [_SG, _I, _T, _T, _P, _P, _P, _P, _P, _P, _P, _T, _T, _P],
    "ea_performer_parts": [_PG],
    "ea_performer_kmax": [_PG, _T, _P, _P, _P],
    "ea_performer_kv": [_PG, _T, _T, _P, _P, _P, _P, _P, _P],
    "ea_performer_out": [_PG, _T, _P, _P, _P, _T, _P],
    "ea_performer_bwd_q": [_PG, _T, _T, _T, _P, _P, _P, _T, _P, _P, _P, _P],
    "ea_performer_bwd_qstats": [_PG, _T, _T, _P, _P, _P, _P, _P, _P, _P],
    "ea_performer_bwd_k": [_PG, _T, _T, _P, _P, _P, _P, _P, _T, _T, _P],
    "ea_lara_seglin_groups": [_G],
    "ea_lara_seglin_fwd": [_G, _T, _T] + [_P] * 11,
    "ea_lara_seglin_bwd": [_G, _T, _T] + [_P] * 10 + [_T, _T, _P, _P, _P, _P],
    "ea_lara_seglin_bwd_fin": [_G, _T, _T] + [_P] * 10 + [_T, _T, _P, _P, _P, _P, _P, _P, ctypes.c_int32, ctypes.c_float, _P],
    "ea_lara_fold_fwd": [_I, _I, _I] + [_P] * 11,
    "ea_lara_fold_parts": [_I],
    "ea_lara_fold_bwd": [_I, _I, _P, _P, _P, _P, _P, _L] + [_P] * 10,
    "ea_performer_f32_parts": [_PG],
    "ea_performer_f32_kmax": [_PG, _T, _P, _P, _P],
    "ea_performer_f32_kv": [_PG, _T, _T, _P, _P, _P, _P, _P, _P],
    "ea_performer_f32_out": [_PG, _T, _P, _P, _P, _T, _P],
    "ea_performer_f32_bwd_q": [_PG, _T, _T, _P, _P, _P, _T, _P, _P, _P],
    "ea_performer_f32_bwd_k": [_PG, _T, _T, _P, _P, _P, _P, _P, _T, _T, _P],
    "ea_kernelized_parts": [_KG],
    "ea_kernelized_stats": [_KG, _T, _T, _P, _P, _P],
    "ea_kernelized_kv": [_KG, _T, _T, _P, _P, _P, _P, _P, _P],
    "ea_kernelized_out": [_KG, _T, _P, _P, _P, _P, _T, _P],
    "ea_kernelized_bwd_q": [_KG, _T, _T, _P, _P, _P, _P, _T, _P, _P, _P, _P],
    "ea_kernelized_bwd_k": [_KG, _T, _T, _P, _P, _P, _P, _P, _T, _T, _P, _P],
    "ea_ceva_decode_close": [_DG, _T, _T, _T, _P, _P, _T, _T, _P],
    "ea_ceva_decode_attn": [_DG, _T, _T, _T, _P, _P, _T, _T, _T, _P],
    "ea_ceva_sdecode_append": [_SDG, _P, _P, _P, _P, _P],
    "ea_ceva_sdecode_close": [_SDG, _T, _T, _T, _P, _P, _T, _T, _P],
    "ea_ceva_sdecode_attn": [_SDG, _T, _T, _T, _P, _P, _T, _T, _T, _P],
    "ea_ceva_sdecode_attn_split": [_SDG, _T, _T, _T, _P, _P, _T, _T, _T, _I, _P, _P],
    "ea_ceva_sdecode_close_l16": [_SDG, _T, _T, _T, _P, _P, _T, _T, _P],
    "ea_ceva_sdecode_attn_l16": [_SDG, _T, _T, _T, _P, _P, _T, _T, _T, _P],
    "ea_ceva_sdecode_attn_split_l16": [_SDG, _T, _T, _T, _P, _P, _T, _T, _T, _I, _P, _P],
    "ea_ceva_sdecode_merge": [_SDG, _T, _I, _P, _P],
    "ea_ceva_sdecode_advance": [_SDG, _P],
    "ea_ceva_sdecode_linear": [_I, _I, _I, _P, _I, _L, _P, _I, _P, _P, _I, _L, _P],
    "ea_ceva_sdecode_linear_fused": [_I, _I, _I, _P, _I, _L, _P, _P, _F, _P, _I, _P, _I, _P, _I, _L, _P, _I, _L, _P],
    "ea_softmax_attn_fwd": [_I, _I, _I, _I, _I, _F, _T, _T, _T, _P, _T, _P, _P, _F, _I, _P],
    "ea_softmax_sample": [_I, _I, _I, _I, _I, _F, _T, _T, _P, _P, _P],
# ... 157 lines not shown
```

### efficient-attention_amd/efficient_attention/_ops.py

```python
import ctypes
import math
import os
import threading
import warnings

import torch
import torch.nn.functional as F

from . import _native as nv

KERNEL_TIMER = nv.KERNEL_TIMER
_DIRECT = os.environ.get("EA_DIRECT_IMPL", "1") == "1"


def _ea_op(name, impl, *args):
    if _DIRECT and not torch.compiler.is_compiling() and torch._C._len_torch_dispatch_stack() == 0:
        return impl(*args)
    return getattr(torch.ops.ea, name)(*args)


def landmark_flops(BH, L, C, D, has_mlp, mixed, eva, bwd):
    f = 0
    if not bwd:
        if has_mlp:
# ... 1264 lines not shown
    pp = [nv.ptr(t) for t in ps] if has_mlp else [None] * 8
    if isinstance(d_omega, tuple):
        _, dom_q, p_domk, S_, scale_ = d_omega
        nv.call_as("ea_lara_landmarks_bwd", "ea_lara_landmarks_bwd_parts", ctypes.byref(lg), nv.ptr(pq), nv.ptr(pk), *pp, nv.ptr(noise_c),
                nv.ptr(dom_q), S_, nv.ptr(p_domk), scale_, nv.ptr(d_qrows), nv.ptr(d_bhv), nv.ptr(d_lp), nv.ptr(dpq),
                nv.ptr(dpk), nv.ptr(dW), nv.ptr(dvec), nv.ptr(saved), nv.stream())
    else:
        nv.call("ea_lara_landmarks_bwd", ctypes.byref(lg), nv.ptr(pq), nv.ptr(pk), *pp, nv.ptr(noise_c),
                nv.ptr(d_omega), nv.ptr(d_qrows), nv.ptr(d_bhv), nv.ptr(d_lp), nv.ptr(dpq), nv.ptr(dpk),
                nv.ptr(dW), nv.ptr(dvec), nv.ptr(saved), nv.stream())
    fin_ = []
    if defer_finish:
        fin_ = [("finish", dict(B=B, gh=H, gw=W, r=r, C=C, scale=float(fcfg[1]), uq=uq, dpq=dpq, dpk=dpk,
                                qbar=qrows if uq is not None else None, lse_t=lse_t if uq is not None else None))]
    else:
        _lara_finish(geom, qkv5, dqkv5, qrows, uq, lse_t, dpq, dpk, (r, H, W))
    grads = [dqkv5]
    if has_mlp and defer_param_sums:
        return grads + [("partials", dW.view(BH, -1), dvec.view(BH, -1))] + fin_
    if has_mlp:
        grads += _mlp_grads(*colsum2_f32(dW.view(BH, -1), dvec.view(BH, -1)), d)
    return grads + fin_


class LaraPooledFn(torch.autograd.Function):

    @staticmethod
    def forward(ctx, qkv5, mask_u8, noise, cfg, *params):
        H, W, r, has_mlp, mixed, mis, dup, kappa, scale = cfg
        icfg = [int(H), int(W), int(r), int(bool(has_mlp)), int(bool(mixed)), int(mis), int(dup),
                int(any(ctx.needs_input_grad))]
        fcfg = [float(kappa), float(scale)]
        outs = _ea_op("lara_fwd", lara_fwd_impl, qkv5, mask_u8, noise, icfg, fcfg, list(params))
        ctx.save_for_backward(qkv5, mask_u8, noise, *outs[1:], *params)
        ctx.icfg, ctx.fcfg, ctx.nsaved = icfg, fcfg, len(outs) - 1
        ctx.pdtypes = [t.dtype for t in params]
        return outs[0]

    @staticmethod
    def backward(ctx, dout):
        qkv5, mask_u8, noise, *rest = ctx.saved_tensors
        saved, params = rest[:ctx.nsaved], rest[ctx.nsaved:]
        grads = _ea_op("lara_bwd", lara_bwd_impl, dout, qkv5, mask_u8, noise, list(saved), ctx.icfg, ctx.fcfg, list(params))
        pgrads = [g.to(dt) for g, dt in zip(grads[1:], ctx.pdtypes)]
        return (grads[0], None, None, None) + tuple(pgrads)


USE_PROJ_POOL = os.environ.get("EA_PROJ_POOL", "1") == "1"
USE_MULTI_SUM = os.environ.get("EA_MULTI_SUM", "1") == "1"


def proj_pool_supported(x2, w32, cdtype, B, H, W, r, heads):
    C = x2.shape[1]
    return (USE_PROJ_POOL and heads == 3 and C == 192 and tuple(w32.shape) == (576, 192) and w32.dtype == torch.float32
            and x2.shape[0] == B * H * W and x2.is_contiguous()
            and bool(nv.lib().ea_linear_pool_supported(192, 576, B, H, W, r)))


def project_qkv_pooled(x2, wq, bq32, cdtype, want_cast, B, H, W, r, pq, pk, w_cast=None):
    rows, K = x2.shape
    a_f32 = x2.dtype == torch.float32
    y = torch.empty((rows, 576), dtype=cdtype, device=x2.device)
    a_cast = torch.empty((rows, K), dtype=cdtype, device=x2.device) if (a_f32 and want_cast) else None
    label = "ea_linear_w32_pool"
    if nv.KERNEL_TIMER.enabled:
        label = "ea_linear[192->576,%s->16,+pool]" % ("f32" if a_f32 else "16")
        _note_bytes(label, rows * (K * x2.element_size() + 576 * 2 + (K * 2 if a_cast is not None else 0)))
    nv.call_as(label, "ea_linear_w32_pool", _ELEM[cdtype], B, H, W, r, K, 576, nv.ptr(x2), int(a_f32), x2.stride(0), nv.ptr(wq),
               nv.ptr(bq32), nv.ptr(y), 576, nv.ptr(a_cast), nv.ptr(pq), nv.ptr(pk), nv.ptr(w_cast), nv.stream())
    return y, a_cast


USE_W192 = os.environ.get("EA_W192_PREPARE", "1") == "1"


def w192_usable(wq, wp, cdtype):
    return (USE_W192 and _DIRECT and not torch.compiler.is_compiling() and torch._C._len_torch_dispatch_stack() == 0
            and cdtype in _ELEM and wq.is_cuda and wq.dtype == torch.float32 and wp.dtype == torch.float32
            and tuple(wq.shape) == (576, 192) and tuple(wp.shape) == (192, 192) and wq.is_contiguous() and wp.is_contiguous()
            and (wq.storage_offset() * 4) % 16 == 0 and (wp.storage_offset() * 4) % 16 == 0)


def prepare_w192(wq, wp, cdtype):
    dev = wq.device
    w16q = torch.empty((576, 192), dtype=cdtype, device=dev)
    wsw = torch.empty((576 * 192,), dtype=cdtype, device=dev)
    w16p = torch.empty((192, 192), dtype=cdtype, device=dev)
    w16pT = torch.empty((192, 192), dtype=cdtype, device=dev)
    nv.call("ea_linear_w192_prepare", _ELEM[cdtype], nv.ptr(wq.detach()), nv.ptr(wp.detach()), nv.ptr(w16q), nv.ptr(wsw),
            nv.ptr(w16p), nv.ptr(w16pT), nv.stream())
    return w16q, wsw, w16p, w16pT


def project_qkv_wsw(x2, wsw, w16q, bq32, cdtype, want_cast, grid=None, pq=None, pk=None):
    rows, K = x2.shape
    a_f32 = x2.dtype == torch.float32
    if grid is None and rows < 65536:
        y, ac = ea_linear(x2, w16q, bq32, cdtype, want_cast)
        return y, ac
    y = torch.empty((rows, 576), dtype=cdtype, device=x2.device)
    a_cast = torch.empty((rows, K), dtype=cdtype, device=x2.device) if (a_f32 and want_cast) else None
    B, H, W, r = grid if grid is not None else (0, 0, 0, 0)
    label = "ea_linear_wsw"
    if nv.KERNEL_TIMER.enabled:
        label = "ea_linear[192->576,%s->16%s]" % ("f32" if a_f32 else "16", ",+pool" if grid is not None else "")
        _note_bytes(label, rows * (K * x2.element_size() + 576 * 2 + (K * 2 if a_cast is not None else 0)))
    nv.call_as(label, "ea_linear_wsw", _ELEM[cdtype], rows, B, H, W, r, nv.ptr(x2), int(a_f32), x2.stride(0), nv.ptr(wsw),
               nv.ptr(bq32), nv.ptr(y), 576, nv.ptr(a_cast), nv.ptr(pq), nv.ptr(pk), nv.stream())
    return y, a_cast


USE_CORE_MODULE_FN = os.environ.get("EA_CORE_MODULE_FN", "1") == "1"


class SoftmaxCore:
    n_inputs = 0

    def __init__(self, mask_u8, keep=None, keep_scale=1.0):
        self.mask_u8, self.keep, self.keep_scale = mask_u8, keep, float(keep_scale)

    def fwd(self, qkv5, inputs):
        out, lse = softmax_fwd_impl(qkv5, self.mask_u8, self.keep, self.keep_scale)
        return out, (lse,)

    def bwd(self, dout, qkv5, out, saved):
        return softmax_bwd_impl(dout, qkv5, self.mask_u8, out, saved[0], self.keep, self.keep_scale), ()


class LocalCore:
    n_inputs = 1

    def __init__(self, mask_u8, attn_2d, seq_shape, window, ext, tb=None):
        self.mask_u8, self.geo = mask_u8, _geo(attn_2d, seq_shape, window, ext)
        self.bias_cols = 0
        self.tb = tb

    def fwd(self, qkv5, inputs):
        bias = inputs[0]
        if self.tb is not None and bias is not None:
            B, N, _, h, d = qkv5.shape
            a2, s0, s1, window, ext = self.geo
            bias = self.tb.dense(bias, self.tb.ld(B, h, N, d, nv.io_dtype(qkv5), bool(a2), (s0, s1) if a2 else (s0,), window, ext))
        self.bias_cols = 0 if bias is None else bias.shape[-1]
        out, lse, bias_p = local_fwd_impl(qkv5, bias, self.mask_u8, self.geo)
        return out, (lse, bias_p)

    def bwd(self, dout, qkv5, out, saved):
        dqkv5, dbias = local_bwd_impl(dout, None, qkv5, _opt(saved[1]), self.mask_u8, out, saved[0], self.geo, self.bias_cols)
        dbias = _opt(dbias)
        if self.tb is not None and dbias is not None:
            dbias = self.tb.grad(dbias)
        return dqkv5, (dbias,)


class PerformerCore:
    n_inputs = 0

    def __init__(self, mask_u8, W):
        self.mask_u8, self.W = mask_u8, W

    def fwd(self, qkv5, inputs):
        out, p_max, kv, ksum = performer_f32_fwd(qkv5, self.mask_u8, self.W)
        return out, (p_max, kv, ksum)

    def bwd(self, dout, qkv5, out, saved):
        return performer_f32_bwd(dout, qkv5, self.mask_u8, self.W, saved[0], saved[1], saved[2]), ()


USE_LARA_1D_MODULE_FN = os.environ.get("EA_LARA_1D_MODULE_FN", "1") == "1"
USE_CAUSAL_MODULE_FN = os.environ.get("EA_CAUSAL_MODULE_FN", "1") == "1"
EVA_1D_NO_MASK = os.environ.get("EA_EVA_1D_NO_MASK", "1") == "1"
USE_GRAPH_CORE = os.environ.get("EA_GRAPH_CORE", "1") == "1"


# ... 97 lines not shown
            parts = _mlp_partials(g[2]) + ([("dbias", g[2][3], g[2][4])] if len(g[2]) > 3 else [])
            extra = extra[:1]
        return g[0], extra, parts, fin

    def scatter(self, res, extra):
        dbias, pgrads = extra[0], extra[1:]
        if "mlp_W" in res:
            pgrads = _mlp_grads(res["mlp_W"][0], res["mlp_v"][0], self.dims[2])
        if "dbias" in res:
            dbias = res["dbias"][0].view(res["dbias"][1])[..., :self.bias_cols].contiguous()
        if dbias is not None and self.tb is not None:
            dbias = self.tb.grad(dbias)
        return [dbias] + pgrads


class LaraCore:
    defers = True

    def __init__(self, mask_u8, noise, cfg):
        self.mask_u8, self.noise, self.cfg = mask_u8, noise, cfg

    def setup(self, B, N, heads, d, elem, inputs, need_grad):
        H, W, r, has_mlp, mixed, mis, dup, kappa, scale = self.cfg
        self.icfg = [int(H), int(W), int(r), int(bool(has_mlp)), int(bool(mixed)), int(mis), int(dup), int(need_grad)]
        self.fcfg = [float(kappa), float(scale)]
        self.dims, self.pooled = (B, heads, d, elem), None

    def project(self, x2, wq, bq32, cdtype, want, need_dx, w192):
        H, W, r = self.icfg[:3]
        B, heads, d, elem = self.dims
        if not proj_pool_supported(x2, wq, cdtype, B, H, W, r, heads):
            return None
        sizes = _lara_layer_cfg_dims(B, heads, d, elem, self.icfg, self.fcfg)[1] if _lara_use_composite() else None
        ws, pq, pk = _pooled_rows(sizes, 3, B * heads, (H // r) * (W // r), d, x2.device)
        self.pooled = (ws, None, None) if ws is not None else (None, pq, pk)
        return _project_qkv_grid(x2, wq, bq32, cdtype, want, need_dx, w192, (B, H, W, r), pq, pk)

    def fwd(self, qkv5, inputs):
        pooled, self.pooled = self.pooled, None
        if pooled is not None:
            outs = lara_fwd_impl(qkv5, self.mask_u8, self.noise, self.icfg, self.fcfg, list(inputs), pooled=pooled)
        else:
            outs = _ea_op("lara_fwd", lara_fwd_impl, qkv5, self.mask_u8, self.noise, self.icfg, self.fcfg, list(inputs))
        self.nsaved = len(outs) - 1
        return outs[0], tuple(outs[1:]) + tuple(inputs)

    def bwd(self, dout, qkv5, out, saved, defer, fin_ok):
        saved, params = saved[:self.nsaved], saved[self.nsaved:]
        args = (dout, qkv5, self.mask_u8, self.noise, list(saved), self.icfg, self.fcfg, list(params))
        if not defer:
            g = _ea_op("lara_bwd", lara_bwd_impl, *args)
            return g[0], g[1:], (), None
        H, W, r = self.icfg[:3]
        use_fin = bool(fin_ok and self.icfg[6] == 0 and (H // r) * (W // r) <= 64)
        g = lara_bwd_impl(*args, defer_param_sums=True, defer_finish=use_fin)
        fin = (g.pop()[1], qkv5.view(qkv5.shape[0] * qkv5.shape[1], -1)) if use_fin else None
        if g[1:] and isinstance(g[1], tuple):
            return g[0], [], _mlp_partials(g[1]), fin
        return g[0], g[1:], (), fin

    def scatter(self, res, extra):
        return _mlp_grads(res["mlp_W"][0], res["mlp_v"][0], self.dims[2]) if "mlp_W" in res else extra


class CoreModuleFn(torch.autograd.Function):

    @staticmethod
    def forward(ctx, x, wq, bq, wp, bp, core, cdtype, heads, *inputs):
        B, C = x.shape[0], x.shape[-1]
        N = x.numel() // (B * C)
        d = C // heads
        x2 = x.reshape(-1, C)
        elem = _ELEM[cdtype]
        need = ctx.needs_input_grad
        direct = _DIRECT and not torch.compiler.is_compiling() and torch._C._len_torch_dispatch_stack() == 0
        lin = linear_w32_impl if direct else torch.ops.ea.linear_w32
        if hasattr(core, "setup"):
            core.setup(B, N, heads, d, elem, inputs, any(need))
        bq32 = None if bq is None else (bq if bq.dtype == torch.float32 else bq.float())
        bp32 = None if bp is None else (bp if bp.dtype == torch.float32 else bp.float())
        want = x2.dtype == torch.float32 and need[1]
        lib = module_proj_lib(C)
        w16q = w16p = b16p = None
        w192 = prepare_w192(wq, wp, cdtype) if (not lib and w192_usable(wq, wp, cdtype)) else None
        w16pT = None if w192 is None else w192[3]
        if lib:
            w16q, b16q, w16p, b16p = lib_casts(wq, bq, wp, bp, cdtype)
            y, xc = lib_project(x2, wq, bq32, w16q, b16q, cdtype)
            want = True
        else:
            project = getattr(core, "project", None) if direct else None
            done = None if project is None else project(x2, wq, bq32, cdtype, want, need[0], w192)
            if done is not None:
                y, xc, w16q = done
            elif w192 is not None:
                w16q = w192[0]
                y, xc = project_qkv_wsw(x2, w192[1], w16q, bq32, cdtype, want)
            else:
                y, xc = lin(x2, wq, bq32, elem, False, False, want)
        xl = x2 if x2.dtype == cdtype else (xc if want else None)
        qkv5 = y.view(B, N, 3, heads, d)
        out, saved = core.fwd(qkv5, inputs)
        o2 = out.reshape(-1, C)
        if lib:
            with torch.autocast(device_type="cuda", enabled=False):
                y2 = F.linear(o2, w16p, b16p)
        elif w192 is not None:
            y2 = ea_linear(o2, w192[2], bp32, cdtype)[0]
        else:
            y2 = lin(o2, wp, bp32, elem, False, False, False)[0]
        ctx.save_for_backward(xl, qkv5, o2, wq, wp, w16q, w16p, w16pT, *saved)
        ctx.core = core
        ctx.meta = (x.shape, x.dtype, cdtype, None if bq is None else bq.dtype, None if bp is None else bp.dtype, wq.dtype, wp.dtype,
                    heads, [None if t is None else t.dtype for t in inputs])
        return y2.view(x.shape)

    @staticmethod
    def backward(ctx, dy):
        xl, qkv5, o2, wq, wp, w16q, w16p, w16pT, *saved = ctx.saved_tensors
        xshape, xdtype, cdtype, bqd, bpd, wqd, wpd, heads, in_dtypes = ctx.meta
        core = ctx.core
        C = xshape[-1]
        d = C // heads
        need = ctx.needs_input_grad
        if need[1] and xl is None:
            raise RuntimeError("%s: the weight gradient was requested but the forward did not keep its input"
                               % ctx._forward_cls.__name__)
        direct = _DIRECT and not torch.compiler.is_compiling() and torch._C._len_torch_dispatch_stack() == 0
        dy2 = dy.reshape(-1, C)
        if dy2.dtype != cdtype:
            dy2 = dy2.to(cdtype)
        if w16p is not None:
            dy2 = dy2 if dy2.is_contiguous() else dy2.contiguous()
            d_o2 = dy2 @ w16p
        elif w16pT is not None and _lin_rows_ok(dy2, cdtype):
            d_o2 = ea_linear(dy2, w16pT, None, cdtype)[0]
        else:
            lin = linear_w32_impl if direct else torch.ops.ea.linear_w32
            d_o2 = lin(dy2, wp, None, _ELEM[cdtype], True, False, False)[0]
        defer = direct and USE_MULTI_SUM
        need_bq, need_bp = bqd is not None and need[2], bpd is not None and need[4]
        qkv2 = qkv5.view(-1, 3 * C)
        pair = bool(defer and need[1] and need[3] and wgrad_pair_usable(qkv2, xl, dy2, o2))
        dwq = dbq = dwp = dbp = dx = None
        pend = []
        if need[3] and not pair:
            r_ = wgrad(dy2, o2, need_bp, defer=defer)
            if defer:
                pend.append(("proj", r_[0], r_[1]))
            else:
                dwp, dbp = r_[0].to(wpd), (r_[1].to(bpd) if need_bp else None)
        elif need_bp and not pair:
            dbp = bias_grad(dy2 if dy2.is_contiguous() else dy2.contiguous()).to(bpd)
        B, N = qkv5.shape[:2]
        dout, out = d_o2.view(B, N, heads, d), o2.view(B, N, heads, d)
        if getattr(core, "defers", False):
            dqkv5, extra, parts, fin = core.bwd(dout, qkv5, out, saved, defer,
                                                bool(need[0] and dgrad_finish_usable(qkv2, wq, xdtype, heads, d)))
            pend += parts
        else:
            (dqkv5, extra), fin = core.bwd(dout, qkv5, out, saved), None
        dqkv2 = dqkv5.view(-1, 3 * C)
        if fin is not None:
            dx = qkv_dgrad_finish(dqkv2, fin[1], wq, w16q, xdtype, fin[0]).view(xshape)
        if pair:
            rq, rp = wgrad_pair(dqkv2, xl, need_bq, dy2, o2, need_bp)
            pend += [("qkv", rq[0], rq[1]), ("proj", rp[0], rp[1])]
        elif need[1]:
            r_ = wgrad(dqkv2, xl, need_bq, defer=defer)
            if defer:
                pend.append(("qkv", r_[0], r_[1]))
            else:
                dwq, dbq = r_[0].to(wqd), (r_[1].to(bqd) if need_bq else None)
        elif need_bq:
            dbq = bias_grad(dqkv2).to(bqd)
        if need[0] and dx is None:
            dx = qkv_dgrad(dqkv2, wq, w16q, xdtype).view(xshape)
        res = {}
        if pend:
            sums = multi_sum([t for _, t, _ in pend])
            res = {what: (o, meta) for (what, _, meta), o in zip(pend, sums)}
            if "proj" in res:
                dwp, dbp = _wgrad_split(*res["proj"])
                dwp, dbp = dwp.to(wpd), (dbp.to(bpd) if need_bp else None)
            if "qkv" in res:
                dwq, dbq = _wgrad_split(*res["qkv"])
                dwq, dbq = dwq.to(wqd), (dbq.to(bqd) if need_bq else None)
        if hasattr(core, "scatter"):
            extra = core.scatter(res, extra)
        egrads = tuple(None if (g is None or dt is None) else g.to(dt) for g, dt in zip(extra, in_dtypes))
        return (dx, dwq, dbq, dwp, dbp, None, None, None) + egrads


class EvaModuleFn(CoreModuleFn):
    """CoreModuleFn around an EvaCore, under the name EVA's single node has in graphs, tests and messages."""


class LaraModuleFn(CoreModuleFn):
    """CoreModuleFn around a LaraCore, under the name LinearRA's single node has in graphs, tests and messages."""


USE_WIDE_MODULE_FN = os.environ.get("EA_WIDE_MODULE_FN", "1") == "1"


def multi_cast(ts, dtype):
    ts = [t.detach() if t.is_contiguous() else t.detach().contiguous() for t in ts]
    outs = [torch.empty(t.shape, dtype=dtype, device=t.device) for t in ts]
    K = len(ts)
    src = (ctypes.c_void_p * K)(*[t.data_ptr() for t in ts])
    dst = (ctypes.c_void_p * K)(*[o.data_ptr() for o in outs])
    n = (ctypes.c_int64 * K)(*[t.numel() for t in ts])
    nv.call("ea_multi_cast", _ELEM[dtype], K, src, n, dst, nv.stream())
    return outs


def module_proj_lib(C):
    return not (_lin_geometry(C, 3 * C) and _lin_geometry(C, C))


def lib_project(x2, w32, b32, w16, b16, cdtype):
    xl = x2 if x2.dtype == cdtype else x2.to(cdtype)
    with torch.autocast(device_type="cuda", enabled=False):
        y = F.linear(xl, w16, b16)
    return y, xl


def lib_casts(wq, bq, wp, bp, cdtype):
    src = [t for t in (wq, bq, wp, bp) if t is not None]
    if all(t.dtype == torch.float32 for t in src):
        cs = multi_cast(src, cdtype)
    else:
        cs = [t if t.dtype == cdtype else t.to(cdtype) for t in src]
    it = iter(cs)
    return tuple(None if t is None else next(it) for t in (wq, bq, wp, bp))


def core_module_fn_supported(x, qkv, proj, cdtype):
    return (USE_CORE_MODULE_FN and _DIRECT and not torch.compiler.is_compiling() and torch._C._len_torch_dispatch_stack() == 0
            and lara_module_fn_supported(x, qkv, proj, cdtype, allow_lib=True))


def lara_module_fn_supported(x, qkv, proj, cdtype, allow_lib=False):
    if not (USE_LARA_MODULE_FN and x.is_cuda and cdtype in _ELEM and x.dtype in (torch.float32, cdtype)):
        return False
    C = x.shape[-1]
    x2 = x.reshape(-1, C)

    def w_ok(w, out):
        return (w.dtype == torch.float32 and w.dim() == 2 and w.is_contiguous() and tuple(w.shape) == (out, C)
                and (w.storage_offset() * 4) % 16 == 0)
    geo = (_lin_geometry(C, 3 * C) and _lin_geometry(C, C)) or (allow_lib and USE_WIDE_MODULE_FN)
    return (w_ok(qkv.weight, 3 * C) and w_ok(proj.weight, C) and _lin_rows_ok(x2, cdtype) and geo
            and USE_WGRAD and C % 64 == 0 and x2.shape[0] >= 64)


def _lmk_saved(geom, device):
    n = nv.lib().ea_lara_landmarks_saved_floats(ctypes.byref(geom))
    if n < 0:
        raise RuntimeError("ea_lara_landmarks_saved_floats: %d" % n)
    return torch.empty(n, dtype=torch.float32, device=device)
# ... 498 lines not shown
def performer_attention(qkv5, mask_u8, proj):
    tracing = torch.compiler.is_compiling() or torch._C._len_torch_dispatch_stack() != 0
    if not PERFORMER_16BIT and (not tracing or qkv5.dtype == torch.float32) and performer_f32_supported(qkv5, proj):
        return PerformerF32Fn.apply(qkv5, mask_u8, proj)
    if qkv5.dtype == torch.float32:
        qkv5 = to_io_dtype(qkv5)
    return PerformerAttnFn.apply(qkv5, mask_u8, proj)


def _split_k(rows):
    best = 1
    for s in range(2, 65):
        if rows % s == 0 and rows // s >= 512:
            best = s
    return best


def _colsum_raw(x2):
    rows, cols = x2.shape
    out = torch.empty(cols, dtype=torch.float32, device=x2.device)
    nv.call("ea_colsum_f32", rows, cols, nv.ptr(x2), nv.ptr(out), nv.stream())
    return out


COLSUM_TWO_STAGE = os.environ.get("EA_COLSUM_TWO_STAGE", "1") == "1"


def _colsum_fold(rows, cols):
    if not COLSUM_TWO_STAGE or cols >= 8192 or rows * cols < (4 << 20):
        return 1
    best = 1
    for k in (64, 32, 16, 12, 8, 4):
        if rows % k == 0 and rows // k >= 64 and k * cols <= 32768:
            best = k
            break
    return best


def colsum_f32(x2):
    rows, cols = x2.shape
    k = _colsum_fold(rows, cols)
    if k > 1:
        return _colsum_raw(_colsum_raw(x2.view(rows // k, k * cols)).view(k, cols))
    return _colsum_raw(x2)


def colsum2_f32(x1, x2):
    rows, c1 = x1.shape
    c2 = x2.shape[1]
    out = torch.empty(c1 + c2, dtype=torch.float32, device=x1.device)
    nv.call_as("ea_colsum_f32", "ea_colsum2_f32", rows, c1, nv.ptr(x1), nv.ptr(out), c2, nv.ptr(x2),
               ctypes.c_void_p(out.data_ptr() + 4 * c1), nv.stream())
    return out[:c1], out[c1:]


def bias_grad(dy2):
    rows, cols = dy2.shape
    if dy2.dtype not in (torch.bfloat16, torch.float16) or cols % 8 or cols > 16384 or not dy2.is_contiguous():
        return dy2.sum(0, dtype=torch.float32)
    nb = nv.lib().ea_bias_grad_parts(rows, cols)
    part = torch.empty(nb * cols, dtype=torch.float32, device=dy2.device)
    db = torch.empty(cols, dtype=torch.float32, device=dy2.device)
    nv.call("ea_bias_grad", 0 if dy2.dtype == torch.bfloat16 else 1, rows, cols, nv.ptr(dy2),
                 nv.ptr(part), nv.ptr(db), nv.stream())
    return db


_MM_OUT_DTYPE = [True]


def _mm_out(a, b, out_dtype):
    if out_dtype == torch.float32 and a.dtype in (torch.bfloat16, torch.float16) and _MM_OUT_DTYPE[0]:
        try:
            return torch.mm(a, b, out_dtype=torch.float32)
        except (TypeError, RuntimeError, NotImplementedError):
            _MM_OUT_DTYPE[0] = False
    return (a @ b).to(out_dtype)


USE_DGRAD_RS = os.environ.get("EA_DGRAD_RS", "1") == "1"
DGRAD_RS_MIN_ROWS = int(os.environ.get("EA_DGRAD_RS_MIN_ROWS", "16384"))


def qkv_dgrad(dqkv2, wq, w16, xdtype):
    rows, NO = dqkv2.shape
    cdtype = dqkv2.dtype
    K = wq.shape[1]
    direct = _DIRECT and not torch.compiler.is_compiling() and torch._C._len_torch_dispatch_stack() == 0
    if (USE_DGRAD_RS and direct and rows >= DGRAD_RS_MIN_ROWS and cdtype in _ELEM and xdtype in (torch.float32, cdtype)
            and tuple(wq.shape) == (NO, K) and dqkv2.stride(1) == 1 and dqkv2.stride(0) % 8 == 0
            and (w16 is not None or wq.dtype == torch.float32)
            and bool(nv.lib().ea_linear_dgrad_supported(K, NO))):
        w = w16 if (w16 is not None and w16.dtype == cdtype and w16.is_contiguous()) else wq
        if w.dtype in (torch.float32, cdtype) and w.is_contiguous():
            dx = torch.empty((rows, K), dtype=xdtype, device=dqkv2.device)
            label = "ea_linear_dgrad"
            if nv.KERNEL_TIMER.enabled:
                label = "ea_linear_dgrad[%d->%d,16->%s]" % (NO, K, "f32" if xdtype == torch.float32 else "16")
                _note_bytes(label, rows * (NO * 2 + K * dx.element_size()))
            nv.call_as(label, "ea_linear_dgrad", _ELEM[cdtype], rows, K, NO, nv.ptr(dqkv2), dqkv2.stride(0), nv.ptr(w),
                       int(w.dtype == torch.float32), nv.ptr(dx), int(xdtype == torch.float32), K, nv.stream())
            return dx
    return _mm_out(dqkv2, w16 if w16 is not None else wq.to(cdtype), xdtype)


USE_DGRAD_FIN = os.environ.get("EA_DGRAD_FIN", "1") == "1"


def dgrad_finish_usable(dqkv2, wq, xdtype, heads, d):
    direct = _DIRECT and not torch.compiler.is_compiling() and torch._C._len_torch_dispatch_stack() == 0
    return (USE_DGRAD_FIN and USE_DGRAD_RS and direct and heads == 3 and d == 64 and dqkv2.dtype in _ELEM
            and xdtype in (torch.float32, dqkv2.dtype) and tuple(wq.shape) == (576, 192) and dqkv2.is_contiguous()
            and dqkv2.shape[0] >= DGRAD_RS_MIN_ROWS)


def qkv_dgrad_finish(dqkv2, qkv2, wq, w16, xdtype, fin):
    rows = dqkv2.shape[0]
    cdtype = dqkv2.dtype
    w = w16 if (w16 is not None and w16.dtype == cdtype and w16.is_contiguous()) else wq
    if not (w.dtype in (torch.float32, cdtype) and w.is_contiguous()):
        w = wq.to(cdtype).contiguous()
    dx = torch.empty((rows, 192), dtype=xdtype, device=dqkv2.device)
    label = "ea_linear_dgrad_finish"
    if nv.KERNEL_TIMER.enabled:
        label = "ea_linear_dgrad_finish[576->192,16->%s%s]" % ("f32" if xdtype == torch.float32 else "16", ",+t" if fin.get("uq") is not None else "")
        _note_bytes(label, rows * (576 * 2 + 384 * 2 + 192 * dx.element_size() + (192 * 2 if fin.get("uq") is not None else 0)))
    nv.call_as(label, "ea_linear_dgrad_finish", _ELEM[cdtype], fin["B"], fin["gh"], fin["gw"], fin["r"], fin["C"], fin["scale"],
               nv.ptr(dqkv2), dqkv2.stride(0), nv.ptr(qkv2), 0 if qkv2 is None else qkv2.stride(0), nv.ptr(w),
               int(w.dtype == torch.float32), nv.ptr(dx), int(xdtype == torch.float32), 192, nv.ptr(fin.get("qbar")),
               nv.ptr(fin.get("uq")), nv.ptr(fin.get("lse_t")), nv.ptr(fin.get("dpq")), nv.ptr(fin.get("dpk")), nv.stream())
    return dx


def slice_sum(part):
    S = part.shape[0]
    n = part[0].numel()
    out = torch.empty(part.shape[1:], dtype=torch.float32, device=part.device)
    nv.call("ea_slice_sum", 1, S, n, 1.0, None, nv.ptr(part), nv.ptr(out), nv.stream())
    return out


USE_EA_LINEAR = os.environ.get("EA_LINEAR", "1") == "1"
LABEL_ALGO_BYTES = {}


def _note_bytes(label, nbytes):
    rec = LABEL_ALGO_BYTES.setdefault(label, [0, 0])
    rec[0] += nbytes
    rec[1] += 1
_ELEM = {torch.bfloat16: 0, torch.float16: 1}


def _lin_geometry(K, NO):
    if K not in (64, 128, 192, 256):
        return False
    for ns in (1, 2, 3, 4):
        if NO % ns == 0 and NO // ns in (64, 128, 192, 256) and (NO // ns) * K * 2 <= 72 * 1024:
            return True
    return False


def _lin_rows_ok(a2, wdtype):
    return (USE_EA_LINEAR and a2.is_cuda and a2.dim() == 2 and a2.stride(1) == 1 and a2.stride(0) % 8 == 0
            and a2.shape[0] > 0 and (a2.storage_offset() * a2.element_size()) % 16 == 0
            and a2.dtype in (wdtype, torch.float32))


def ea_linear_supported(a2, w):
    return (w.dtype in _ELEM and w.is_contiguous() and _lin_rows_ok(a2, w.dtype)
            and _lin_geometry(w.shape[1], w.shape[0]))


def linear_impl(a2, w, bias32, y_f32, want_cast):
    nv.require_cuda(a2, "a")
    y, ac = ea_linear(a2, w, bias32, torch.float32 if y_f32 else w.dtype, want_cast)
    return [y, ac if ac is not None else a2.new_empty(0, dtype=w.dtype)]


_ELEM_DT = [torch.bfloat16, torch.float16]


def linear_w32_impl(a2, w32, bias32, elem, transposed, y_f32, want_cast):
    nv.require_cuda(a2, "a")
    dt = _ELEM_DT[int(elem)]
    y, ac = ea_linear(a2, w32, bias32, torch.float32 if y_f32 else dt, want_cast, elem_dtype=dt, transposed=bool(transposed))
    return [y, ac if ac is not None else a2.new_empty(0, dtype=dt)]


def ea_linear_w32_supported(a2, w32, dtype, transposed=False):
    K, NO = (w32.shape[0], w32.shape[1]) if transposed else (w32.shape[1], w32.shape[0])
    return (dtype in _ELEM and w32.dtype == torch.float32 and w32.is_contiguous() and w32.dim() == 2
            and (w32.storage_offset() * 4) % 16 == 0 and _lin_rows_ok(a2, dtype) and a2.shape[1] == K and _lin_geometry(K, NO))


def ea_linear(a2, w, bias32, out_dtype, want_cast=False, elem_dtype=None, transposed=False):
    rows, K = a2.shape
    w32 = elem_dtype is not None
    cdt = elem_dtype if w32 else w.dtype
    NO = w.shape[1] if (w32 and transposed) else w.shape[0]
    y = torch.empty((rows, NO), dtype=out_dtype, device=a2.device)
    a_f32 = a2.dtype == torch.float32
    a_cast = torch.empty((rows, K), dtype=cdt, device=a2.device) if (a_f32 and want_cast) else None
    label = "ea_linear"
    if nv.KERNEL_TIMER.enabled:
        label = "ea_linear[%d->%d,%s->%s]" % (K, NO, "f32" if a_f32 else "16", "f32" if out_dtype == torch.float32 else "16")
        _note_bytes(label, rows * (K * a2.element_size() + NO * y.element_size() + (K * 2 if a_cast is not None else 0)))
    if w32:
        nv.call_as(label, "ea_linear_w32", _ELEM[cdt], rows, K, NO, nv.ptr(a2), int(a_f32), a2.stride(0), nv.ptr(w),
                   int(transposed), nv.ptr(bias32), nv.ptr(y), int(out_dtype == torch.float32), NO, nv.ptr(a_cast), nv.stream())
    else:
        nv.call_as(label, "ea_linear", _ELEM[cdt], rows, K, NO, nv.ptr(a2), int(a_f32), a2.stride(0), nv.ptr(w), nv.ptr(bias32),
                   nv.ptr(y), int(out_dtype == torch.float32), NO, nv.ptr(a_cast), nv.stream())
# ... 369 lines not shown
```

### include/ea_hip.h

```cpp
#ifndef EA_HIP_H
#define EA_HIP_H

#include <stdint.h>

#ifdef __cplusplus
extern "C" {
#endif

#define EA_BF16 0
#define EA_F16  1
#define EA_F32  2

#define EA_OK            0
#define EA_E_BADARG     -1
#define EA_E_UNSUPPORTED -2

typedef struct {
  void*   ptr;
  int64_t sb, sh, sn;
} ea_t4;

typedef struct {
  int32_t B, H, N, D;
  int32_t dtype;
// ... 221 lines not shown
                      const float* p_m2, const float* kv, const float* qbar,
                      float* r, float* dbh, float* dlp, float* dkk, float* dkv, float* domq,
                      float* dqbar, float* uq, void* stream);

int ea_bias_grad_parts(int32_t rows, int32_t cols);
int ea_bias_grad(int32_t dtype, int32_t rows, int32_t cols, const void* dy, float* part, float* db,
                 void* stream);

int ea_colsum_f32(int32_t rows, int32_t cols, const float* x, float* out, void* stream);
int ea_colsum2_f32(int32_t rows, int32_t cols1, const float* x1, float* out1, int32_t cols2, const float* x2, float* out2,
                   void* stream);
int ea_gather_sum(int32_t rows, int32_t K, int32_t cols, const float* g, const int32_t* inv, float* out, void* stream);
int ea_table_bias_fwd(int32_t h, int32_t th, int32_t Wq, int32_t Wk, int32_t ld, float scale, const float* table, const int32_t* idx,
                      float* out, void* stream);
int ea_table_bias_bwd(int32_t rows, int32_t K, int32_t h, int32_t Wq, int32_t Wk, int32_t ld, float scale, const float* g,
                      const int32_t* inv, float* dtable, void* stream);
int ea_multi_cast(int32_t dtype, int32_t K, const float* const* src, const int64_t* n, void* const* dst, void* stream);
int ea_slice_sum(int32_t BH, int32_t S, int32_t n, float scale, const float* a, const float* parts,
                 float* out, void* stream);
int ea_stream_copy(const void* src, void* dst, int64_t bytes, void* stream);

int ea_lara_segment_fwd(const ea_geom* g, const ea_t4* q2, const ea_t4* k2, const uint8_t* mask,
                        const float* bias_q, const float* bias_k, const float* mbias_q, const float* mbias_k,
                        const float* gq, const float* cq, const float* gk, const float* ck,
                        float* qbar, float* kbar, void* stream);
int ea_lara_segment_bwd(const ea_geom* g, const ea_t4* q2, const ea_t4* k2, const uint8_t* mask,
                        const float* bias_q, const float* bias_k, const float* mbias_q, const float* mbias_k,
                        const float* gq, const float* cq, const float* gk, const float* ck,
                        const float* d_qbar, const float* d_kbar, const ea_t4* dq2, const ea_t4* dk2,
                        float* part, void* stream);

int32_t ea_rows_mlp_parts(int32_t R, int32_t D);
int ea_rows_mlp_fwd(int32_t R, int32_t D, int32_t sides, int32_t layer_norm,
                    const float* x0, const float* x1, const float* W0, const float* W1,
                    const float* b0, const float* b1, const float* g0, const float* g1,
                    const float* c0, const float* c1, float* y0, float* y1,
                    float* zhat, float* rstd, void* stream);
int ea_rows_mlp_bwd(int32_t R, int32_t D, int32_t sides, int32_t layer_norm,
                    const float* dy0, const float* dy1, const float* x0, const float* x1,
                    const float* W0, const float* W1, const float* g0, const float* g1,
                    const float* zhat, const float* rstd, float* dx0, float* dx1,
                    float* feed, float* dW_part, void* stream);

int32_t ea_wgrad_parts(int32_t rows, int32_t out_features, int32_t in_features);
int ea_wgrad(int32_t dtype, int32_t rows, int32_t out_features, int32_t in_features, const void* dy, const void* x,
             float* dw_part, float* db_part, int64_t part_ld, void* stream);
int ea_part_sum(int32_t S, int32_t n, int64_t ld, const float* parts, float* out, void* stream);
int32_t ea_wgrad_pair_parts(int32_t rows, int32_t out1, int32_t in1, int32_t out2, int32_t in2);
int ea_wgrad_pair(int32_t dtype, int32_t rows, int32_t out1, int32_t in1, const void* dy1, const void* x1, float* dw_part1,
                  float* db_part1, int64_t part_ld1, int32_t out2, int32_t in2, const void* dy2, const void* x2,
                  float* dw_part2, float* db_part2, int64_t part_ld2, void* stream);
int ea_multi_sum(int32_t K, const float* const* parts, const int32_t* S, const int32_t* n, const int64_t* ld, float* const* out,
                 void* stream);

int ea_lara_sample_fwd(int32_t BH, int32_t L, int32_t C, int32_t D, int32_t mis, int32_t mode, float scale,
                       const float* qbar, const float* mu, const float* noise, float* omega, float* qbar_rows, float* bhv,
                       float* lp, void* stream);
int ea_lara_sample_bwd(int32_t BH, int32_t L, int32_t C, int32_t D, int32_t mis, int32_t mode, float scale,
                       const float* qbar, const float* mu, const float* noise, const float* d_omega, const float* d_qbar_rows,
                       const float* d_bhv, const float* d_lp, float* d_qbar, float* d_mu, void* stream);

int ea_adaptive_pool2d_fwd(int32_t dtype, int32_t B, int32_t H, int32_t gh, int32_t gw, int32_t side, int32_t D,
                           const ea_t4* x, float* mean, void* stream);
int ea_adaptive_pool2d_bwd(int32_t dtype, int32_t B, int32_t H, int32_t gh, int32_t gw, int32_t side, int32_t D,
                           const float* dmean, const ea_t4* dx, void* stream);

int32_t ea_linear_supported(int32_t in_features, int32_t out_features);
int ea_linear(int32_t dtype, int32_t rows, int32_t in_features, int32_t out_features, const void* a, int32_t a_f32,
              int64_t lda, const void* w, const float* bias, void* y, int32_t y_f32, int64_t ldy, void* a_cast,
              void* stream);
int ea_linear_w32(int32_t dtype, int32_t rows, int32_t in_features, int32_t out_features, const void* a, int32_t a_f32,
                  int64_t lda, const float* w, int32_t w_transposed, const float* bias, void* y, int32_t y_f32, int64_t ldy,
                  void* a_cast, void* stream);
int32_t ea_linear_pool_supported(int32_t in_features, int32_t out_features, int32_t B, int32_t gh, int32_t gw, int32_t r);
int ea_linear_w32_pool(int32_t dtype, int32_t B, int32_t gh, int32_t gw, int32_t r, int32_t in_features, int32_t out_features,
                       const void* a, int32_t a_f32, int64_t lda, const float* w, const float* bias, void* y, int64_t ldy,
                       void* a_cast, float* pooled_q, float* pooled_k, void* w_cast, void* stream);

int ea_linear_w192_prepare(int32_t dtype, const float* wq, const float* wp, void* w16q, void* wq_sw, void* w16p, void* w16pT,
                           void* stream);
int ea_linear_wsw(int32_t dtype, int32_t rows, int32_t B, int32_t gh, int32_t gw, int32_t r, const void* a, int32_t a_f32, int64_t lda,
                  const void* wq_sw, const float* bias, void* y, int64_t ldy, void* a_cast, float* pooled_q, float* pooled_k,
                  void* stream);

int32_t ea_linear_dgrad_supported(int32_t in_features, int32_t out_features);
int ea_linear_dgrad(int32_t dtype, int32_t rows, int32_t in_features, int32_t out_features, const void* dy, int64_t ldy,
                    const void* w, int32_t w_f32, void* dx, int32_t dx_f32, int64_t ldx, void* stream);

int ea_linear_dgrad_finish(int32_t dtype, int32_t B, int32_t gh, int32_t gw, int32_t pool_r, int32_t C, float scale,
                           void* dqkv, int64_t ldy, const void* qkv, int64_t ldq, const void* w, int32_t w_f32, void* dx,
                           int32_t dx_f32, int64_t ldx, const float* qbar, const float* uq, const float* lse_t,
                           const float* dpq, const float* dpk, void* stream);

int ea_lara_out_fwd_merge(const ea_lara_geom* g, const ea_t4* q, const float* omega, const float* qbar, const float* bhv,
                          int32_t S, const float* p_ml, const float* p_kv, const float* lp, float* kv, float* lse_k,
                          float* lse_t, float* cst, const ea_t4* out, float* lseZ, float* tmean, void* stream);
int ea_lara_bwd_k_fused_merge(const ea_lara_geom* g, const ea_t4* k, const ea_t4* v, const uint8_t* mask, const float* omega,
                              const float* qbar, const float* kv, const float* lse_k, int32_t S, const float* p_ml,
                              const float* p_dkv, const float* p_dom, const float* p_m1, const float* p_m2,
                              const ea_t4* dk, const ea_t4* dv, float* p_domk, float* dbh, float* dlp, float* domq,
                              float* dqbar, float* uq, void* stream);
int ea_lara_landmarks_bwd_parts(const ea_lmk_geom* g, const float* pq, const float* pk,
                                const float* Wq, const float* bq, const float* gq, const float* cq,
                                const float* Wk, const float* bk, const float* gk, const float* ck,
                                const float* noise, const float* d_omega, int32_t dom_S, const float* dom_parts, float dom_scale,
                                const float* d_qbar_rows, const float* d_bhv, const float* d_lp, float* dpq, float* dpk,
                                float* dW_part, float* dvec_part, const float* saved, void* stream);

typedef struct {
  int32_t B, H, Nq, Nk, D;
  int32_t G, Wq, Wk, L;
  int32_t knorm;
  int32_t neg_inf, causal_e, chunk, lm_base;
  int32_t bias_ld;
  int64_t bias_hs, bias_bs, keep_ld;
  float   keep_scale, scale;
} ea_f32_attn;
int ea_f32_attn_fwd(const ea_f32_attn* g, const ea_t4* q, const ea_t4* k, const ea_t4* v, const ea_t4* ek, const ea_t4* ev,
                    const int32_t* idx_q, const int32_t* idx_k, const float* bias, const uint8_t* kmask, const uint8_t* qmask,
                    const uint8_t* keep, const ea_t4* out, float* lse, float* stat, void* stream);
int ea_f32_attn_bwd(const ea_f32_attn* g, const ea_t4* q, const ea_t4* k, const ea_t4* v, const ea_t4* ek, const ea_t4* ev,
                    const int32_t* idx_q, const int32_t* idx_k, const float* bias, const uint8_t* kmask, const uint8_t* qmask,
                    const uint8_t* keep, const ea_t4* out, const ea_t4* dout, const float* stat, const float* dlse,
                    const ea_t4* dq, float* dk, float* dv, float* dek, float* dev, float* dbias, void* stream);
int ea_f32_gather_mean_fwd(int32_t B, int32_t H, int32_t N, int32_t D, int32_t Cn, int32_t J, const ea_t4* x, const int32_t* idx,
                           const uint8_t* mask, float* mean, void* stream);
int ea_f32_gather_mean_bwd(int32_t B, int32_t H, int32_t N, int32_t D, int32_t Cn, int32_t J, const int32_t* idx,
                           const uint8_t* mask, const float* dmean, float* dx, void* stream);

typedef struct {
  int32_t B, H, D;
  int32_t dtype;
  int32_t gh, gw;
  int32_t pool_r;
  int32_t has_mlp, mixed, mis, dup;
  float   kappa, scale;
} ea_lara_layer;
#define EA_LARA_POOLED_READY 2
int64_t ea_lara_layer_ws(const ea_lara_layer* cfg, int32_t which);
int ea_lara_layer_fwd(const ea_lara_layer* cfg, const ea_t4* q, const ea_t4* k, const ea_t4* v, const uint8_t* mask,
                      const float* noise, const float* const* params, const ea_t4* out, float* saved, float* tmp,
                      int32_t keep_for_backward, void* stream);
int ea_lara_layer_bwd(const ea_lara_layer* cfg, const ea_t4* q, const ea_t4* k, const ea_t4* v, const uint8_t* mask,
                      const float* noise, const float* const* params, const ea_t4* dout, const ea_t4* dq, const ea_t4* dk,
                      const ea_t4* dv, const float* saved, float* tmp, float* dparams, void* stream);
#define EA_LARA_DEFER_FINISH 1
int ea_lara_layer_bwd2(const ea_lara_layer* cfg, const ea_t4* q, const ea_t4* k, const ea_t4* v, const uint8_t* mask,
                       const float* noise, const float* const* params, const ea_t4* dout, const ea_t4* dq, const ea_t4* dk,
                       const ea_t4* dv, const float* saved, float* tmp, float* dparams, int32_t flags, void* stream);

typedef struct {
  int32_t B, H, D;
  int32_t dtype;
  int32_t gh, gw;
  int32_t window;
  int32_t chunk;
  int32_t has_bias;
  float   scale;
} ea_eva_layer;
int64_t ea_eva_layer_ws(const ea_eva_layer* cfg, int32_t which);
int ea_eva_layer_fwd(const ea_eva_layer* cfg, const ea_t4* q, const ea_t4* k, const ea_t4* v, const float* bias,
                     const float* noise, const float* const* params, const ea_t4* out, float* saved,
                     int32_t keep_for_backward, void* stream);
int ea_eva_layer_bwd(const ea_eva_layer* cfg, const ea_t4* q, const ea_t4* k, const ea_t4* v, const float* bias,
                     const float* noise, const float* const* params, const ea_t4* out, const ea_t4* dout, const ea_t4* dq,
                     const ea_t4* dk, const ea_t4* dv, const float* saved, float* tmp, float* dbias, float* dparams,
// ... 113 lines not shown
```

Before: 202.4 million tokens/s.

## Pre-swizzle transposed QKV weight for dgrad and switch LDS tiles to psi swizzle

Adds a prepared transposed, per-lane-swizzled bf16 image of the QKV weight, built in the w192 prepare kernel, so the dgrad and dgrad-finish kernels load their register weight fragments with one coalesced 16-byte load per k-step instead of gathering from the row-major weight. It also replaces the LDS swizzle in the proj and dgrad tiles with a new psi permutation to cut bank conflicts, and reworks the tile-store and pool index math around it. The cost is an extra 576x192 weight buffer written each forward and an ABI bump.

```diff
diff --git a/efficient-attention_amd/csrc/ea_capi.hip b/efficient-attention_amd/csrc/ea_capi.hip
--- a/efficient-attention_amd/csrc/ea_capi.hip
+++ b/efficient-attention_amd/csrc/ea_capi.hip
@@ -33,7 +33,8 @@
 int proj_rs_dispatch(int dtype, const void* a, int a_f32, const float* w, const float* bias, void* y, void* a_cast, int rows,
                      long lda, long ldy, hipStream_t st, int B, int gh, int gw, int r, float* pq, float* pk, void* w_cast,
                      const void* wsw);
-int w192_prepare_dispatch(int dtype, const float* wq, const float* wp, void* w16q, void* wsw, void* w16p, void* w16pT, hipStream_t st);
+int w192_prepare_dispatch(int dtype, const float* wq, const float* wp, void* w16q, void* wsw, void* w16p, void* w16pT, void* wtsw,
+                          hipStream_t st);
 int dgrad_rs_supported(int K, int NO);
 int dgrad_fin_launch(int dtype, const void* dqkv, long ldy, const void* qkv, long ldq, const void* w, int w_f32, void* dx, int dx_f32,
                      long ldx, int B, int gh, int gw, int pool_r, int C, float scale, const float* qbar, const float* uq,
@@ -75,7 +76,7 @@
 extern "C" {
 
 const char* ea_version(void) { return "ea_hip 0.1.0 gfx950"; }
-int32_t ea_abi_version(void) { return 24; }
+int32_t ea_abi_version(void) { return 25; }
 
 int32_t ea_window_bias_ld(const ea_geom* g) {
   WinTiling t;
@@ -1447,7 +1448,16 @@
       ((uintptr_t)w16p & 15) || ((uintptr_t)w16pT & 15))
     return EA_E_BADARG;
   if (wp && (!w16p || !w16pT)) return EA_E_BADARG;
-  return w192_prepare_dispatch(dtype, wq, wp, w16q, wq_sw, w16p, w16pT, (hipStream_t)stream);
+  return w192_prepare_dispatch(dtype, wq, wp, w16q, wq_sw, w16p, w16pT, nullptr, (hipStream_t)stream);
+}
+
+int ea_linear_w192_prepare_t(int32_t dtype, const float* wq, const float* wp, void* w16q, void* wq_sw, void* w16p, void* w16pT,
+                             void* wqT_sw, void* stream) {
+  if (!wq || !w16q || !wq_sw || !wqT_sw || ((uintptr_t)wq & 15) || ((uintptr_t)wp & 15) || ((uintptr_t)w16q & 15) ||
+      ((uintptr_t)wq_sw & 15) || ((uintptr_t)w16p & 15) || ((uintptr_t)w16pT & 15) || ((uintptr_t)wqT_sw & 15))
+    return EA_E_BADARG;
+  if (wp && (!w16p || !w16pT)) return EA_E_BADARG;
+  return w192_prepare_dispatch(dtype, wq, wp, w16q, wq_sw, w16p, w16pT, wqT_sw, (hipStream_t)stream);
 }
 
 int ea_linear_wsw(int32_t dtype, int32_t rows, int32_t B, int32_t gh, int32_t gw, int32_t r, const void* a, int32_t a_f32, int64_t lda,
diff --git a/efficient-attention_amd/csrc/ea_common.h b/efficient-attention_amd/csrc/ea_common.h
--- a/efficient-attention_amd/csrc/ea_common.h
+++ b/efficient-attention_amd/csrc/ea_common.h
@@ -2,6 +2,7 @@
 #include <hip/hip_runtime.h>
 #include <stdint.h>
 #include "../../include/ea_hip.h"
+#include "ea_lds_swizzle.h"
 
 #ifdef EA_PROFILE
 #include <stdio.h>
@@ -273,10 +274,15 @@
   }
 };
 
-EA_DEV int phi2(int row) { return (((row >> 1) & 3) << 1) | ((row ^ (row >> 3)) & 1); }
+EA_DEV int phi2(int row) { return swz_phi2(row); }
 template <int D> EA_DEV int lds_off2(int row, int chunk16) {
   static_assert(D == 64, "lds_off2: 128-byte rows only");
   return row * (D * 2) + ((chunk16 ^ phi2(row)) << 4);
+}
+EA_DEV int psi(int row) { return swz_psi(row); }
+template <int D> EA_DEV int lds_off3(int row, int chunk16) {
+  static_assert(D == 64, "lds_off3: 128-byte rows only");
+  return row * (D * 2) + ((chunk16 ^ psi(row)) << 4);
 }
 template <int D> struct LaneOff2 {
   static constexpr int ROWB = D * 2, KS = D / 32, DT = D / 16;
diff --git a/efficient-attention_amd/csrc/ea_dgrad_rs.hip b/efficient-attention_amd/csrc/ea_dgrad_rs.hip
--- a/efficient-attention_amd/csrc/ea_dgrad_rs.hip
+++ b/efficient-attention_amd/csrc/ea_dgrad_rs.hip
@@ -17,10 +17,13 @@
 constexpr int DG_PIECE = 32 * DG_NO * 2;
 constexpr int DG_LDS = 2 * DG_TILE;
 
-EA_DEV int dg_off(int slab, int tok, int chunk16) { return slab * (DG_TOK * 128) + lds_off2<64>(tok, chunk16); }
-
-template <typename E, bool WF32, bool OF32>
-__global__ __launch_bounds__(DG_WAVES * 64, 3) void dgrad_rs_kernel(const DgP p) {
+EA_DEV int dg_off(int slab, int tok, int chunk16) { return slab * (DG_TOK * 128) + lds_off3<64>(tok, chunk16); }
+
+EA_DEV size_t dg_wt_off(int wave, int ks, int lane) { return ((size_t)(wave * DG_KT + ks) * 64 + lane) * 16; }
+
+template <typename E, bool WF32, bool OF32, bool WT>
+EA_DEV void dgrad_rs_body(const DgP& p) {
+  static_assert(!(WT && WF32), "the prepared image is in the element type");
   extern __shared__ __attribute__((aligned(16))) char smem[];
   char* const tile0 = smem;
   char* const tile1 = smem + DG_TILE;
@@ -44,7 +47,10 @@
   int t = blockIdx.x;
   if (t < p.ntiles) issue(t);
   typename E::x8 wr[DG_KT];
-  {
+  if constexpr (WT) {
+#pragma unroll
+    for (int ks = 0; ks < DG_KT; ++ks) wr[ks] = as_x8<E>(ldg16(p.w + dg_wt_off(wave, ks, lane)));
+  } else {
     const int o_l = tid / 24, c = tid - o_l * 24;
     const int rho = ((o_l >> 2) & 1) * 16 + (o_l >> 3) * 4 + (o_l & 3);
     const int wofs = rho * (DG_NO * 2) + c * 16;
@@ -111,6 +117,11 @@
     }
   }
 }
+
+template <typename E, bool WF32, bool OF32>
+__global__ __launch_bounds__(DG_WAVES * 64, 3) void dgrad_rs_kernel(const DgP p) { dgrad_rs_body<E, WF32, OF32, false>(p); }
+template <typename E, bool OF32>
+__global__ __launch_bounds__(DG_WAVES * 64, 3) void dgrad_rs_wt_kernel(const DgP p) { dgrad_rs_body<E, false, OF32, true>(p); }
 
 struct DgFinP {
   DgP d;
@@ -130,8 +141,9 @@
 constexpr int DG_LMR = 64 * 128;
 constexpr int DG_FIN_LDS = 2 * DG_TILE + 2 * DG_QT + 6 * DG_LMR + 3 * 64 * 4;
 
-template <typename E, bool WF32, bool OF32, bool HAS_T, bool POOL, int PR>
-__global__ __launch_bounds__(DG_WAVES * 64, 3) void dgrad_fin_kernel(const DgFinP p) {
+template <typename E, bool WF32, bool OF32, bool HAS_T, bool POOL, int PR, bool WT>
+EA_DEV void dgrad_fin_body(const DgFinP& p) {
+  static_assert(!(WT && WF32), "the prepared image is in the element type");
   static_assert(PR == 0 || (POOL && (PR == 2 || PR == 4)), "cell-major order needs 2 x 2 or 4 x 4 pooling cells");
   constexpr int TPC = PR * PR, CPT = PR ? DG_TOK / (PR * PR) : 1;
   extern __shared__ __attribute__((aligned(16))) char smem[];
@@ -146,7 +158,10 @@
   constexpr bool pool = POOL;
   EA_BLK(p.d, 0);
   typename E::x8 wr[DG_KT];
-  {
+  if constexpr (WT) {
+#pragma unroll
+    for (int ks = 0; ks < DG_KT; ++ks) wr[ks] = as_x8<E>(ldg16(p.d.w + dg_wt_off(wave, ks, lane)));
+  } else {
     const int o_l = tid / 24, c = tid - o_l * 24;
     const int rho = ((o_l >> 2) & 1) * 16 + (o_l >> 3) * 4 + (o_l & 3);
     const int wofs = rho * (DG_NO * 2) + c * 16;
@@ -395,10 +410,20 @@
   EA_BLK(p.d, 1);
 }
 
+template <typename E, bool WF32, bool OF32, bool HAS_T, bool POOL, int PR>
+__global__ __launch_bounds__(DG_WAVES * 64, 3) void dgrad_fin_kernel(const DgFinP p) {
+  dgrad_fin_body<E, WF32, OF32, HAS_T, POOL, PR, false>(p);
+}
+template <typename E, bool OF32, bool HAS_T, bool POOL, int PR>
+__global__ __launch_bounds__(DG_WAVES * 64, 3) void dgrad_fin_wt_kernel(const DgFinP p) {
+  dgrad_fin_body<E, false, OF32, HAS_T, POOL, PR, true>(p);
+}
+
 int dgrad_rs_supported(int K, int NO) { return K == DG_K && NO == DG_NO; }
 
-int dgrad_rs_dispatch(int dtype, const void* dy, const void* w, int w_f32, void* dx, int dx_f32, int rows, long ldy, long ldx,
+int dgrad_rs_dispatch(int dtype, const void* dy, const void* w, int w_kind, void* dx, int dx_f32, int rows, long ldy, long ldx,
                       hipStream_t st) {
+  if (w_kind < 0 || w_kind > 2) return EA_E_BADARG;
   if (rows <= 0) return EA_OK;
   DgP p = {};
   p.dy = (const char*)dy; p.w = (const char*)w; p.dx = (char*)dx;
@@ -411,21 +436,29 @@
     EA_SET_LDS_ONCE((&dgrad_rs_kernel<E_, WF_, OF_>), DG_LDS);                            \
     hipLaunchKernelGGL((dgrad_rs_kernel<E_, WF_, OF_>), g, b, DG_LDS, st, p);             \
   } while (0)
+#define EA_DG_LAUNCH_WT(E_, OF_)                                                          \
+  do {                                                                                    \
+    EA_SET_LDS_ONCE((&dgrad_rs_wt_kernel<E_, OF_>), DG_LDS);                              \
+    hipLaunchKernelGGL((dgrad_rs_wt_kernel<E_, OF_>), g, b, DG_LDS, st, p);               \
+  } while (0)
 #define EA_DG_SEL(E_)                                                                     \
   do {                                                                                    \
-    if (w_f32) { if (dx_f32) EA_DG_LAUNCH(E_, true, true); else EA_DG_LAUNCH(E_, true, false); }   \
+    if (w_kind == 2) { if (dx_f32) EA_DG_LAUNCH_WT(E_, true); else EA_DG_LAUNCH_WT(E_, false); }   \
+    else if (w_kind) { if (dx_f32) EA_DG_LAUNCH(E_, true, true); else EA_DG_LAUNCH(E_, true, false); }   \
     else { if (dx_f32) EA_DG_LAUNCH(E_, false, true); else EA_DG_LAUNCH(E_, false, false); }       \
   } while (0)
   if (dtype == EA_BF16) EA_DG_SEL(BF16);
   else if (dtype == EA_F16) EA_DG_SEL(F16);
   else return EA_E_BADARG;
 #undef EA_DG_SEL
+#undef EA_DG_LAUNCH_WT
 #undef EA_DG_LAUNCH
   return (int)hipGetLastError();
 }
 
-int dgrad_fin_dispatch(int dtype, const DgFinP& p0, int w_f32, int dx_f32, bool has_t, int pr, hipStream_t st) {
+int dgrad_fin_dispatch(int dtype, const DgFinP& p0, int w_kind, int dx_f32, bool has_t, int pr, hipStream_t st) {
   DgFinP p = p0;
+  if (w_kind < 0 || w_kind > 2) return EA_E_BADARG;
   if (p.d.rows <= 0) return EA_OK;
   int grid = ea_device_cus();
   if (grid > p.nunits) grid = p.nunits;
@@ -434,10 +467,20 @@
   ProfReport rep;
   p.d.prof = rep.arm(st, "dgrad_fin", pr);
 #endif
-#define EA_DF_LAUNCH(E_, WF_, OF_, T_, P_, R_)                                                    \
+#define EA_DF_LAUNCH_W(E_, WF_, OF_, T_, P_, R_)                                                  \
   do {                                                                                            \
     EA_SET_LDS_ONCE((&dgrad_fin_kernel<E_, WF_, OF_, T_, P_, R_>), DG_FIN_LDS);                   \
     hipLaunchKernelGGL((dgrad_fin_kernel<E_, WF_, OF_, T_, P_, R_>), g, b, DG_FIN_LDS, st, p);    \
+  } while (0)
+#define EA_DF_LAUNCH_WT(E_, OF_, T_, P_, R_)                                                      \
+  do {                                                                                            \
+    EA_SET_LDS_ONCE((&dgrad_fin_wt_kernel<E_, OF_, T_, P_, R_>), DG_FIN_LDS);                     \
+    hipLaunchKernelGGL((dgrad_fin_wt_kernel<E_, OF_, T_, P_, R_>), g, b, DG_FIN_LDS, st, p);      \
+  } while (0)
+#define EA_DF_LAUNCH(E_, WF_, OF_, T_, P_, R_)                                                    \
+  do {                                                                                            \
+    if constexpr (WF_ == 2) EA_DF_LAUNCH_WT(E_, OF_, T_, P_, R_);                                 \
+    else EA_DF_LAUNCH_W(E_, (WF_ == 1), OF_, T_, P_, R_);                                         \
   } while (0)
 #define EA_DF_SEL3(E_, WF_, OF_, T_)                                                          \
   do {                                                                                        \
@@ -453,8 +496,9 @@
   } while (0)
 #define EA_DF_SEL(E_)                                                                     \
   do {                                                                                    \
-    if (w_f32) { if (dx_f32) EA_DF_SEL2(E_, true, true); else EA_DF_SEL2(E_, true, false); }   \
-    else { if (dx_f32) EA_DF_SEL2(E_, false, true); else EA_DF_SEL2(E_, false, false); }       \
+    if (w_kind == 2) { if (dx_f32) EA_DF_SEL2(E_, 2, true); else EA_DF_SEL2(E_, 2, false); }   \
+    else if (w_kind) { if (dx_f32) EA_DF_SEL2(E_, 1, true); else EA_DF_SEL2(E_, 1, false); }   \
+    else { if (dx_f32) EA_DF_SEL2(E_, 0, true); else EA_DF_SEL2(E_, 0, false); }               \
   } while (0)
   if (dtype == EA_BF16) EA_DF_SEL(BF16);
   else if (dtype == EA_F16) EA_DF_SEL(F16);
@@ -463,10 +507,12 @@
 #undef EA_DF_SEL2
 #undef EA_DF_SEL3
 #undef EA_DF_LAUNCH
+#undef EA_DF_LAUNCH_W
+#undef EA_DF_LAUNCH_WT
   return (int)hipGetLastError();
 }
 
-int dgrad_fin_launch(int dtype, const void* dqkv, long ldy, const void* qkv, long ldq, const void* w, int w_f32, void* dx, int dx_f32,
+int dgrad_fin_launch(int dtype, const void* dqkv, long ldy, const void* qkv, long ldq, const void* w, int w_kind, void* dx, int dx_f32,
                      long ldx, int B, int gh, int gw, int pool_r, int C, float scale, const float* qbar, const float* uq,
                      const float* lse_t, const float* dpq, const float* dpk, hipStream_t st) {
   DgFinP p = {};
@@ -497,7 +543,7 @@
     p.m_cw = (unsigned)((1ull << 32) / (unsigned)p.cw) + 1u;
   }
   p.nunits = B * p.splits;
-  return dgrad_fin_dispatch(dtype, p, w_f32, dx_f32, uq != nullptr, pr, st);
-}
-
-}
+  return dgrad_fin_dispatch(dtype, p, w_kind, dx_f32, uq != nullptr, pr, st);
+}
+
+}
diff --git a/efficient-attention_amd/csrc/ea_lds_swizzle.h b/efficient-attention_amd/csrc/ea_lds_swizzle.h
--- /dev/null
+++ b/efficient-attention_amd/csrc/ea_lds_swizzle.h
@@ -0,0 +1,12 @@
+#pragma once
+
+namespace ea {
+
+constexpr int swz_phi2(int row) { return (((row >> 1) & 3) << 1) | ((row ^ (row >> 3)) & 1); }
+
+constexpr int swz_psi(int row) { return ((row >> 1) ^ (row & ~1)) & 7; }
+
+constexpr int swz_off2(int row, int chunk16) { return row * 128 + ((chunk16 ^ swz_phi2(row)) << 4); }
+constexpr int swz_off3(int row, int chunk16) { return row * 128 + ((chunk16 ^ swz_psi(row)) << 4); }
+
+}
diff --git a/efficient-attention_amd/csrc/ea_proj_rs.hip b/efficient-attention_amd/csrc/ea_proj_rs.hip
--- a/efficient-attention_amd/csrc/ea_proj_rs.hip
+++ b/efficient-attention_amd/csrc/ea_proj_rs.hip
@@ -20,7 +20,7 @@
 
 constexpr int RS_K = 192, RS_NO = 576, RS_WAVES = 12, RS_TOK = 32, RS_KT = RS_K / 32, RS_SLABS = RS_K / 64;
 
-EA_DEV int rs_off(int slab, int tok, int chunk16) { return slab * (RS_TOK * 128) + lds_off2<64>(tok, chunk16); }
+EA_DEV int rs_off(int slab, int tok, int chunk16) { return slab * (RS_TOK * 128) + lds_off3<64>(tok, chunk16); }
 
 EA_DEV int rs_col(int wave, int j, int li) {
   const int c0 = 48 * wave;
@@ -83,7 +83,6 @@
           stg16(p.w_cast + ((size_t)col[j] * RS_K + ks * 32 + 8 * g) * 2, __builtin_bit_cast(u32x4, wr[j][ks]));
       }
   }
-  const int slab_s = st_c >> 3, ch_s = st_c & 7;
   constexpr int NC = POOL ? RS_TOK / POOL : 1;
   constexpr int XB = 8 * RS_K * 2;
   __shared__ __attribute__((aligned(16))) char xbar[POOL ? 2 : 1][POOL ? 2 * XB : 16];
@@ -91,8 +90,10 @@
   auto pool_x = [&](int b_) {
     const int slab = wave >> 2, dt = wave & 3;
     const char* tb = tile[b_] + slab * (RS_TOK * 128);
-    const int r_ = 4 * g + (li >> 2);
-    const int off = lds_off2<64>(r_, 2 * dt + ((li & 3) >> 1)) + 8 * (li & 1);
+    int lane_x = lane;
+    asm volatile("" : "+v"(lane_x));
+    const int r_ = lane_x >> 2;
+    const int off = lds_off3<64>(r_, 2 * dt + ((lane_x & 3) >> 1)) + 8 * (lane_x & 1);
     const typename E::x8 a = as_x8<E>(E::tr4(tb + off), E::tr4(tb + 16 * 128 + off));
     const uint32_t one = (uint32_t)E::from_f(1.f) * 0x00010001u;
     const uint32_t lo_on = (POOL == 16 ? li == 0 : li == g) ? one : 0u, hi_on = (POOL == 16 ? li == 1 : li == 4 + g) ? one : 0u;
@@ -149,7 +150,12 @@
       } else {
         w8 = nb[0];
       }
-      sts16(tile[buf] + rs_off(slab_s, st_tok, ch_s), w8);
+      {
+        int tid_s = tid;
+        asm volatile("" : "+v"(tid_s));
+        const int tk = tid_s / 24, c = tid_s - tk * 24;
+        sts16(tile[buf] + rs_off(c >> 3, tk, c & 7), w8);
+      }
       if (AF32 && p.a_cast) {
         const int tok = tok_of(t, st_tok);
         stg16(p.a_cast + ((size_t)tok * RS_K + st_c * 8) * 2, w8);
@@ -225,8 +231,9 @@
 template <typename E>
 __global__ __launch_bounds__(256) void w192_prepare_kernel(const float* __restrict__ wq, const float* __restrict__ wp,
                                                             char* __restrict__ w16q, char* __restrict__ wsw,
-                                                            char* __restrict__ w16p, char* __restrict__ w16pT) {
-  constexpr int NQ = RS_WAVES * 3 * RS_KT * 64, NP = RS_K * RS_K / 8;
+                                                            char* __restrict__ w16p, char* __restrict__ w16pT,
+                                                            char* __restrict__ wtsw) {
+  constexpr int NQ = RS_WAVES * 3 * RS_KT * 64, NP = RS_K * RS_K / 8, NT = 12 * (RS_NO / 32) * 64;
   const int i = blockIdx.x * 256 + threadIdx.x;
   if (i < NQ) {
     const int lane = i & 63, pc = i >> 6, ks = pc % RS_KT, wj = pc / RS_KT, j = wj % 3, wave = wj / 3;
@@ -250,15 +257,23 @@
       t[(size_t)(c * 8 + 2 * q) * RS_K + row] = (uint16_t)(w8[q] & 0xffffu);
       t[(size_t)(c * 8 + 2 * q + 1) * RS_K + row] = (uint16_t)(w8[q] >> 16);
     }
+  } else if (i >= NQ + NP && i < NQ + NP + NT && wtsw) {
+    const int k = i - NQ - NP, lane = k & 63, pc = k >> 6, ks = pc % (RS_NO / 32), wave = pc / (RS_NO / 32);
+    const int g = lane >> 4, li = lane & 15;
+    const float* src = wq + (size_t)(32 * ks + 8 * g) * RS_K + 16 * wave + li;
+    float f[8];
+#pragma unroll
+    for (int q = 0; q < 8; ++q) f[q] = src[(size_t)q * RS_K];
+    stg16(wtsw + (size_t)k * 16, pack8<E>(f));
   }
 }
 
 int w192_prepare_dispatch(int dtype, const float* wq, const float* wp, void* w16q, void* wsw, void* w16p, void* w16pT,
-                          hipStream_t st) {
-  constexpr int N = RS_WAVES * 3 * RS_KT * 64 + RS_K * RS_K / 8;
+                          void* wtsw, hipStream_t st) {
+  const int N = RS_WAVES * 3 * RS_KT * 64 + RS_K * RS_K / 8 + (wtsw ? 12 * (RS_NO / 32) * 64 : 0);
   const dim3 g((N + 255) / 256), b(256);
-  if (dtype == EA_BF16) hipLaunchKernelGGL(w192_prepare_kernel<BF16>, g, b, 0, st, wq, wp, (char*)w16q, (char*)wsw, (char*)w16p, (char*)w16pT);
-  else if (dtype == EA_F16) hipLaunchKernelGGL(w192_prepare_kernel<F16>, g, b, 0, st, wq, wp, (char*)w16q, (char*)wsw, (char*)w16p, (char*)w16pT);
+  if (dtype == EA_BF16) hipLaunchKernelGGL(w192_prepare_kernel<BF16>, g, b, 0, st, wq, wp, (char*)w16q, (char*)wsw, (char*)w16p, (char*)w16pT, (char*)wtsw);
+  else if (dtype == EA_F16) hipLaunchKernelGGL(w192_prepare_kernel<F16>, g, b, 0, st, wq, wp, (char*)w16q, (char*)wsw, (char*)w16p, (char*)w16pT, (char*)wtsw);
   else return EA_E_BADARG;
   return (int)hipGetLastError();
 }
diff --git a/efficient-attention_amd/efficient_attention/_native.py b/efficient-attention_amd/efficient_attention/_native.py
--- a/efficient-attention_amd/efficient_attention/_native.py
+++ b/efficient-attention_amd/efficient_attention/_native.py
@@ -16,7 +16,7 @@
                 ("sn", ctypes.c_int64)]
 
 
-ABI_VERSION = 24
+ABI_VERSION = 25
 
 
 class ea_geom(ctypes.Structure):
@@ -158,6 +158,7 @@
     "ea_table_bias_fwd": [_I, _I, _I, _I, _I, _F, _P, _P, _P, _P],
     "ea_multi_cast": [_I, _I, _P, _P, _P, _P],
     "ea_linear_w192_prepare": [_I, _P, _P, _P, _P, _P, _P, _P],
+    "ea_linear_w192_prepare_t": [_I, _P, _P, _P, _P, _P, _P, _P, _P],
     "ea_linear_wsw": [_I, _I, _I, _I, _I, _I, _P, _I, _L, _P, _P, _P, _L, _P, _P, _P, _P],
     "ea_table_bias_bwd": [_I, _I, _I, _I, _I, _I, _F, _P, _P, _P, _P],
     "ea_linear_supported": [_I, _I],
diff --git a/efficient-attention_amd/efficient_attention/_ops.py b/efficient-attention_amd/efficient_attention/_ops.py
--- a/efficient-attention_amd/efficient_attention/_ops.py
+++ b/efficient-attention_amd/efficient_attention/_ops.py
@@ -1370,14 +1370,27 @@
 
 
 def prepare_w192(wq, wp, cdtype):
+    return _prepare_w192(wq, wp, cdtype, False)
+
+
+def prepare_w192_t(wq, wp, cdtype):
+    return _prepare_w192(wq, wp, cdtype, True)
+
+
+def _prepare_w192(wq, wp, cdtype, with_t):
     dev = wq.device
     w16q = torch.empty((576, 192), dtype=cdtype, device=dev)
     wsw = torch.empty((576 * 192,), dtype=cdtype, device=dev)
     w16p = torch.empty((192, 192), dtype=cdtype, device=dev)
     w16pT = torch.empty((192, 192), dtype=cdtype, device=dev)
-    nv.call("ea_linear_w192_prepare", _ELEM[cdtype], nv.ptr(wq.detach()), nv.ptr(wp.detach()), nv.ptr(w16q), nv.ptr(wsw),
-            nv.ptr(w16p), nv.ptr(w16pT), nv.stream())
-    return w16q, wsw, w16p, w16pT
+    if not with_t:
+        nv.call("ea_linear_w192_prepare", _ELEM[cdtype], nv.ptr(wq.detach()), nv.ptr(wp.detach()), nv.ptr(w16q), nv.ptr(wsw),
+                nv.ptr(w16p), nv.ptr(w16pT), nv.stream())
+        return w16q, wsw, w16p, w16pT
+    wtsw = torch.empty((576 * 192,), dtype=cdtype, device=dev)
+    nv.call("ea_linear_w192_prepare_t", _ELEM[cdtype], nv.ptr(wq.detach()), nv.ptr(wp.detach()), nv.ptr(w16q), nv.ptr(wsw),
+            nv.ptr(w16p), nv.ptr(w16pT), nv.ptr(wtsw), nv.stream())
+    return w16q, wsw, w16p, w16pT, wtsw
 
 
 def project_qkv_wsw(x2, wsw, w16q, bq32, cdtype, want_cast, grid=None, pq=None, pk=None):
@@ -1641,7 +1654,7 @@
         want = x2.dtype == torch.float32 and need[1]
         lib = module_proj_lib(C)
         w16q = w16p = b16p = None
-        w192 = prepare_w192(wq, wp, cdtype) if (not lib and w192_usable(wq, wp, cdtype)) else None
+        w192 = prepare_w192_t(wq, wp, cdtype) if (not lib and w192_usable(wq, wp, cdtype)) else None
         w16pT = None if w192 is None else w192[3]
         if lib:
             w16q, b16q, w16p, b16p = lib_casts(wq, bq, wp, bp, cdtype)
@@ -1668,7 +1681,8 @@
             y2 = ea_linear(o2, w192[2], bp32, cdtype)[0]
         else:
             y2 = lin(o2, wp, bp32, elem, False, False, False)[0]
-        ctx.save_for_backward(xl, qkv5, o2, wq, wp, w16q, w16p, w16pT, *saved)
+        wqT = w192[4] if (w192 is not None and w16q is w192[0]) else None
+        ctx.save_for_backward(xl, qkv5, o2, wq, wp, w16q, w16p, w16pT, wqT, *saved)
         ctx.core = core
         ctx.meta = (x.shape, x.dtype, cdtype, None if bq is None else bq.dtype, None if bp is None else bp.dtype, wq.dtype, wp.dtype,
                     heads, [None if t is None else t.dtype for t in inputs])
@@ -1676,7 +1690,7 @@
 
     @staticmethod
     def backward(ctx, dy):
-        xl, qkv5, o2, wq, wp, w16q, w16p, w16pT, *saved = ctx.saved_tensors
+        xl, qkv5, o2, wq, wp, w16q, w16p, w16pT, wqT, *saved = ctx.saved_tensors
         xshape, xdtype, cdtype, bqd, bpd, wqd, wpd, heads, in_dtypes = ctx.meta
         core = ctx.core
         C = xshape[-1]
@@ -1721,7 +1735,7 @@
             (dqkv5, extra), fin = core.bwd(dout, qkv5, out, saved), None
         dqkv2 = dqkv5.view(-1, 3 * C)
         if fin is not None:
-            dx = qkv_dgrad_finish(dqkv2, fin[1], wq, w16q, xdtype, fin[0]).view(xshape)
+            dx = qkv_dgrad_finish(dqkv2, fin[1], wq, w16q, xdtype, fin[0], wqT).view(xshape)
         if pair:
             rq, rp = wgrad_pair(dqkv2, xl, need_bq, dy2, o2, need_bp)
             pend += [("qkv", rq[0], rq[1]), ("proj", rp[0], rp[1])]
@@ -1734,7 +1748,7 @@
         elif need_bq:
             dbq = bias_grad(dqkv2).to(bqd)
         if need[0] and dx is None:
-            dx = qkv_dgrad(dqkv2, wq, w16q, xdtype).view(xshape)
+            dx = qkv_dgrad(dqkv2, wq, w16q, xdtype, wqT).view(xshape)
         res = {}
         if pend:
             sums = multi_sum([t for _, t, _ in pend])
@@ -2399,7 +2413,14 @@
 DGRAD_RS_MIN_ROWS = int(os.environ.get("EA_DGRAD_RS_MIN_ROWS", "16384"))
 
 
-def qkv_dgrad(dqkv2, wq, w16, xdtype):
+def _dgrad_weight(wq, w16, wt, cdtype):
+    if wt is not None and wt.dtype == cdtype and wt.is_contiguous() and wt.numel() == 576 * 192:
+        return wt, 2
+    w = w16 if (w16 is not None and w16.dtype == cdtype and w16.is_contiguous()) else wq
+    return w, int(w.dtype == torch.float32)
+
+
+def qkv_dgrad(dqkv2, wq, w16, xdtype, wt=None):
     rows, NO = dqkv2.shape
     cdtype = dqkv2.dtype
     K = wq.shape[1]
@@ -2408,7 +2429,7 @@
             and tuple(wq.shape) == (NO, K) and dqkv2.stride(1) == 1 and dqkv2.stride(0) % 8 == 0
             and (w16 is not None or wq.dtype == torch.float32)
             and bool(nv.lib().ea_linear_dgrad_supported(K, NO))):
-        w = w16 if (w16 is not None and w16.dtype == cdtype and w16.is_contiguous()) else wq
+        w, w_kind = _dgrad_weight(wq, w16, wt, cdtype)
         if w.dtype in (torch.float32, cdtype) and w.is_contiguous():
             dx = torch.empty((rows, K), dtype=xdtype, device=dqkv2.device)
             label = "ea_linear_dgrad"
@@ -2416,7 +2437,7 @@
                 label = "ea_linear_dgrad[%d->%d,16->%s]" % (NO, K, "f32" if xdtype == torch.float32 else "16")
                 _note_bytes(label, rows * (NO * 2 + K * dx.element_size()))
             nv.call_as(label, "ea_linear_dgrad", _ELEM[cdtype], rows, K, NO, nv.ptr(dqkv2), dqkv2.stride(0), nv.ptr(w),
-                       int(w.dtype == torch.float32), nv.ptr(dx), int(xdtype == torch.float32), K, nv.stream())
+                       w_kind, nv.ptr(dx), int(xdtype == torch.float32), K, nv.stream())
             return dx
     return _mm_out(dqkv2, w16 if w16 is not None else wq.to(cdtype), xdtype)
 
@@ -2431,12 +2452,12 @@
             and dqkv2.shape[0] >= DGRAD_RS_MIN_ROWS)
 
 
-def qkv_dgrad_finish(dqkv2, qkv2, wq, w16, xdtype, fin):
+def qkv_dgrad_finish(dqkv2, qkv2, wq, w16, xdtype, fin, wt=None):
     rows = dqkv2.shape[0]
     cdtype = dqkv2.dtype
-    w = w16 if (w16 is not None and w16.dtype == cdtype and w16.is_contiguous()) else wq
+    w, w_kind = _dgrad_weight(wq, w16, wt, cdtype)
     if not (w.dtype in (torch.float32, cdtype) and w.is_contiguous()):
-        w = wq.to(cdtype).contiguous()
+        w, w_kind = wq.to(cdtype).contiguous(), 0
     dx = torch.empty((rows, 192), dtype=xdtype, device=dqkv2.device)
     label = "ea_linear_dgrad_finish"
     if nv.KERNEL_TIMER.enabled:
@@ -2444,7 +2465,7 @@
         _note_bytes(label, rows * (576 * 2 + 384 * 2 + 192 * dx.element_size() + (192 * 2 if fin.get("uq") is not None else 0)))
     nv.call_as(label, "ea_linear_dgrad_finish", _ELEM[cdtype], fin["B"], fin["gh"], fin["gw"], fin["r"], fin["C"], fin["scale"],
                nv.ptr(dqkv2), dqkv2.stride(0), nv.ptr(qkv2), 0 if qkv2 is None else qkv2.stride(0), nv.ptr(w),
-               int(w.dtype == torch.float32), nv.ptr(dx), int(xdtype == torch.float32), 192, nv.ptr(fin.get("qbar")),
+               w_kind, nv.ptr(dx), int(xdtype == torch.float32), 192, nv.ptr(fin.get("qbar")),
                nv.ptr(fin.get("uq")), nv.ptr(fin.get("lse_t")), nv.ptr(fin.get("dpq")), nv.ptr(fin.get("dpk")), nv.stream())
     return dx
 
diff --git a/include/ea_hip.h b/include/ea_hip.h
--- a/include/ea_hip.h
+++ b/include/ea_hip.h
@@ -327,6 +327,8 @@
 int ea_linear_wsw(int32_t dtype, int32_t rows, int32_t B, int32_t gh, int32_t gw, int32_t r, const void* a, int32_t a_f32, int64_t lda,
                   const void* wq_sw, const float* bias, void* y, int64_t ldy, void* a_cast, float* pooled_q, float* pooled_k,
                   void* stream);
+int ea_linear_w192_prepare_t(int32_t dtype, const float* wq, const float* wp, void* w16q, void* wq_sw, void* w16p, void* w16pT,
+                             void* wqT_sw, void* stream);
 
 int32_t ea_linear_dgrad_supported(int32_t in_features, int32_t out_features);
 int ea_linear_dgrad(int32_t dtype, int32_t rows, int32_t in_features, int32_t out_features, const void* dy, int64_t ldy,
```

Result: faster. 206.3 million tokens/s (median of 6 runs) (+2.0%).
